# aptos-labs/keyless-zk-proofs

Measured on AMD Instinct MI355X. Metric: BN254 G1 MSM points/s @2^20 (Groth16 prover hot path), higher is better.
Workload: dtype u64 column accumulators over 9 x 29-bit limbs (256-bit Montgomery integers, v_mad_u64_u32); 1 GPU; BN254 G1 Pippenger MSM, 2^20 random scalars/points per GPU, result XYZZ on host; points_per_gpu=1048576, bases=reference format (Montgomery affine), converted inside every step

## Files before the change

include/k16.h:

```cpp
#ifndef K16_H
#define K16_H

#include <stddef.h>
#include <stdint.h>

#ifdef __cplusplus
extern "C" {
#endif

enum {
    K16_OK             = 0,
    K16_ERR_NO_DEVICE  = -1,
    K16_ERR_HIP        = -2,
    K16_ERR_ARG        = -3,
    K16_ERR_IO         = -4,
    K16_ERR_FORMAT     = -5,
    K16_ERR_CURVE      = -6,
    K16_ERR_BUFFER     = -7,
    K16_ERR_NOMEM      = -8
};

enum { K16_G1 = 0, K16_G2 = 1 };
enum { K16_FQ = 0, K16_FR = 1 };
enum { K16_FQ9 = 2, K16_FR9 = 3, K16_FQ2N = 4,
       K16_FQ2H = 5  };
enum { K16_G1_ENG9 = 2, K16_G2_ENG2N = 3, K16_G2_PAIR = 4  };
#define K16_OP_BOUND_A(k) ((k) << 8)
#define K16_OP_BOUND_B(k) ((k) << 12)
enum { K16_OP_ADD = 0, K16_OP_SUB, K16_OP_NEG, K16_OP_MUL, K16_OP_SQR, K16_OP_TOMONT, K16_OP_FROMMONT,
       K16_OP_LAZY_ADDMUL, K16_OP_LAZY_SUBMUL };
enum { K16_PT_ADD = 0, K16_PT_MADD, K16_PT_DBL,
       K16_PT_MADD_ACC };

typedef struct k16_ctx    k16_ctx;
typedef struct k16_prover k16_prover;

int         k16_runtime_hw_queues(int n);
int         k16_device_count(void);
int         k16_host_threads(void);

int         k16_ctx_create(int device, k16_ctx** out);
int         k16_ctx_create_ex(int device, int stream_offset, k16_ctx** out);
void        k16_ctx_destroy(k16_ctx* ctx);
const char* k16_last_error(const k16_ctx* ctx);
enum { K16_OPT_PIPELINED_MSM = 1, K16_OPT_GRAPHS = 2, K16_OPT_SHARED_GPU = 3, K16_OPT_YIELDING_WAITS = 4 };
int         k16_ctx_set_option(k16_ctx* ctx, int option, int value);
int         k16_sync(k16_ctx* ctx);
void*       k16_stream(k16_ctx* ctx);

int k16_dev_alloc(k16_ctx* ctx, size_t bytes, void** dptr);
int k16_dev_free(k16_ctx* ctx, void* dptr);
int k16_h2d(k16_ctx* ctx, void* dptr, const void* hptr, size_t bytes);
int k16_d2h(k16_ctx* ctx, void* hptr, const void* dptr, size_t bytes);
int k16_host_register(k16_ctx* ctx, void* hptr, size_t bytes);
int k16_host_unregister(k16_ctx* ctx, void* hptr);

int k16_timer_start(k16_ctx* ctx);
int k16_timer_stop(k16_ctx* ctx, float* elapsed_ms);
int k16_kernel_stats_enable(k16_ctx* ctx, int on);
int k16_kernel_stats_reset(k16_ctx* ctx);
int k16_kernel_stats_get(k16_ctx* ctx, const char* name, uint64_t* launches, double* total_ms);

int k16_msm(k16_ctx* ctx, int group, const void* d_bases, const void* d_scalars, uint64_t n, void* h_out_xyzz,
            void* h_out_affine);
int k16_msm_host(k16_ctx* ctx, int group, const void* h_bases, const void* h_scalars, uint64_t n, void* h_out_xyzz,
                 void* h_out_affine);
int k16_msm_enqueue(k16_ctx* ctx, int group, const void* d_bases, const void* d_scalars, uint64_t n);
int k16_msm_finish(k16_ctx* ctx, void* h_out_xyzz, void* h_out_affine);
int k16_msm_finish_group(k16_ctx* ctx, int group, void* h_out_xyzz, void* h_out_affine);
int k16_msm_pending(k16_ctx* ctx);
int k16_msm_abort_all(k16_ctx* ctx);
int k16_msm_bases_prepare(k16_ctx* ctx, int group, const void* d_bases, uint64_t n, void* d_out);
int k16_msm_enqueue_prepared(k16_ctx* ctx, int group, const void* d_prepared, const void* d_scalars, uint64_t n);
int k16_msm_fixed_base_info(uint64_t n, unsigned* c, uint64_t* table_rows);
int k16_msm_fixed_base_prepare(k16_ctx* ctx, int group, const void* d_bases, uint64_t n, void* d_table);
int k16_msm_enqueue_fixed_base(k16_ctx* ctx, int group, const void* d_table, const void* d_scalars, uint64_t n);
typedef struct k16_scalar_classes k16_scalar_classes;
int  k16_msm_zero_row_mask(k16_ctx* ctx, int group, const void* d_rows, uint64_t n, void* d_mask);
int  k16_scalar_classes_create(k16_ctx* ctx, uint64_t max_n, int max_sets, k16_scalar_classes** out);
void k16_scalar_classes_destroy(k16_scalar_classes* cls);
int  k16_scalar_classes_build(k16_ctx* ctx, k16_scalar_classes* cls, const void* d_scalars, uint64_t n,
                              const void* const* d_zero_masks, int n_sets, int64_t n_wide_bound);
int  k16_scalar_classes_counts(k16_ctx* ctx, const k16_scalar_classes* cls, uint32_t* out);
int  k16_msm_enqueue_classified(k16_ctx* ctx, int group, const void* d_prepared, const k16_scalar_classes* cls, int set);
int  k16_msm_set_zero_row_mask(k16_ctx* ctx, const void* d_mask);
int  k16_msm_sort_from_lane(k16_ctx* ctx, int lane, int derive);
#define K16_MSM_LANES 4
int k16_msm_set_lane(k16_ctx* ctx, int lane);
int k16_msm_set_window_bits(k16_ctx* ctx, unsigned c);

typedef struct k16_msm_shards k16_msm_shards;
int         k16_msm_sharded_create(const int* devices, int n_devices, int group, uint64_t n, k16_msm_shards** out);
void        k16_msm_sharded_destroy(k16_msm_shards* s);
int         k16_msm_sharded_count(const k16_msm_shards* s);
int         k16_msm_sharded_range(const k16_msm_shards* s, int shard, uint64_t* lo, uint64_t* hi);
k16_ctx*    k16_msm_sharded_ctx(k16_msm_shards* s, int shard);
const char* k16_msm_sharded_last_error(const k16_msm_shards* s);
int         k16_msm_sharded_set_bases(k16_msm_shards* s, const void* h_bases);
int         k16_msm_sharded_set_bases_device(k16_msm_shards* s, int shard, const void* d_slice);
int         k16_msm_sharded_run(k16_msm_shards* s, const void* h_scalars, void* h_out_xyzz, void* h_out_affine);
int         k16_msm_sharded_run_device(k16_msm_shards* s, const void* const* d_scalars, void* h_out_xyzz, void* h_out_affine);
int         k16_msm_sharded_set_piece_rows(k16_msm_shards* s, uint64_t host_rows, uint64_t device_rows);
int         k16_msm_sharded_last_ms(const k16_msm_shards* s, double* shards_ms, double* fold_ms, double* total_ms);
typedef struct k16_rank_comm k16_rank_comm;
int         k16_rank_comm_unique_id(void* out128);
const char* k16_rank_comm_load_error(void);
int         k16_rank_comm_create(k16_ctx* ctx, int rank, int world, const void* unique_id128, k16_rank_comm** out);
void        k16_rank_comm_destroy(k16_rank_comm* c);
int         k16_rank_comm_allgather_fold(k16_rank_comm* c, int group, const void* h_partial_xyzz, void* h_out_xyzz,
                                         void* h_out_affine);
int         k16_rank_comm_allgather_start(k16_rank_comm* c, int group, const void* h_partial_xyzz);
int         k16_rank_comm_allgather_finish(k16_rank_comm* c, void* h_out_xyzz, void* h_out_affine);

int k16_points_sum(int group, const void* h_parts_xyzz, uint64_t count, void* h_out_xyzz, void* h_out_affine);

int k16_ntt(k16_ctx* ctx, void* d_a, uint64_t n, uint64_t max_domain, int inverse);
int k16_ntt_host(k16_ctx* ctx, void* h_a, uint64_t n, uint64_t max_domain, int inverse);

int k16_synth_points(k16_ctx* ctx, int group, uint64_t start, uint64_t n, void* d_out_affine);
int k16_synth_points_scalars(k16_ctx* ctx, int group, const void* d_scalars, uint64_t n, void* d_out_affine);

int k16_field_op_vec(k16_ctx* ctx, int field, int op, const void* h_a, const void* h_b, void* h_r, uint64_t n);
int k16_point_op_vec(k16_ctx* ctx, int group, int op, const void* h_p1, const void* h_p2, void* h_r, uint64_t n);
int k16_coop_exec(k16_ctx* ctx, const uint8_t* step_class, uint64_t n_steps, const uint64_t* words ,
                  const uint32_t* terms, uint64_t n_terms, uint32_t n_const, uint32_t n_slots, const uint32_t* out_slot ,
                  const uint32_t* const9, const void* h_inputs, uint64_t n, void* h_out);

int  k16_prover_create(k16_ctx* ctx, const char* zkey_path, k16_prover** out);
int  k16_prover_create_mem(k16_ctx* ctx, const void* zkey_bytes, size_t zkey_size, k16_prover** out);
int  k16_prover_create_shared(k16_ctx* ctx, const k16_prover* other, k16_prover** out);
void k16_prover_destroy(k16_prover* p);
int  k16_prover_info(const k16_prover* p, uint32_t* n_vars, uint32_t* n_public, uint32_t* domain_size,
                     uint64_t* n_coefs);
int  k16_prover_prove_file(k16_prover* p, const char* wtns_path, const uint8_t* r_std, const uint8_t* s_std,
                           char* out_json, size_t cap, float* device_ms);
int  k16_prover_prove_file_timed(k16_prover* p, const char* wtns_path, const uint8_t* r_std, const uint8_t* s_std,
                                 char* out_json, size_t cap, float* device_ms, float* prove_wall_ms);
int  k16_prover_prove_mem(k16_prover* p, const void* h_wtns, uint64_t n_vars, const uint8_t* r_std,
                          const uint8_t* s_std, char* out_json, size_t cap, float* device_ms);
int  k16_prover_compact_buffers(k16_prover* p, uint8_t** narrow, uint32_t** wide_idx, uint8_t** wide_val, uint64_t* wide_cap);
int  k16_prover_prove_compact(k16_prover* p, uint64_t n_wide, const uint8_t* r_std, const uint8_t* s_std, char* out_json,
                              size_t cap, float* device_ms);
int  k16_fullprover_prove_mem(const void* fullprover, const void* wtns_values, uint64_t n_values, char* out_json, size_t cap,
                              int* prover_time_ms);
int  k16_fullprover_compact_lease(const void* fullprover, void** lease, uint8_t** narrow, uint32_t** wide_idx,
                                  uint8_t** wide_val, uint64_t* wide_cap, uint32_t* n_vars);
int  k16_fullprover_prove_compact(const void* fullprover, void* lease, uint64_t n_wide, char* out_json, size_t cap,
                                  int* prover_time_ms);
int  k16_fullprover_compact_cancel(const void* fullprover, void* lease);
int  k16_prover_last_h(k16_prover* p, void* h_out);
int  k16_prover_warmup_status(const k16_prover* p);

typedef struct k16_vk k16_vk;
int  k16_vk_create(k16_ctx* ctx, const void* alpha1_g1, const void* beta2_g2, const void* gamma2_g2, const void* delta2_g2,
                   const void* ic_g1, uint32_t n_ic, k16_vk** out);
void k16_vk_destroy(k16_vk* vk);
int  k16_verify_batch(k16_ctx* ctx, const k16_vk* vk, const void* h_proofs, const void* h_inputs, uint64_t n,
                      uint8_t* h_out_ok);
int  k16_verify_coop_gt(k16_ctx* ctx, const k16_vk* vk, const void* h_proofs, const void* h_inputs, uint64_t n, void* h_out_gt);
int  k16_pairing_vec(k16_ctx* ctx, const void* h_g1, const void* h_g2, uint64_t n, void* h_out_gt);

enum { K16_PT_OK = 0, K16_PT_NONCANONICAL = 1, K16_PT_OFF_CURVE = 2, K16_PT_NOT_IN_SUBGROUP = 3 };
enum { K16_VERIFY_PAIRING_MISMATCH = 4 };
int  k16_points_check(k16_ctx* ctx, int group, const void* h_points, uint64_t n, uint8_t* h_status);
int  k16_verify_batch_checked(k16_ctx* ctx, const k16_vk* vk, const void* h_proofs, const void* h_inputs, uint64_t n,
                              uint8_t* h_out_ok, uint8_t* h_out_reason);
#define K16_VERIFY_FOLD_MIN 2049
int  k16_verify_batch_folded(k16_ctx* ctx, const k16_vk* vk, const void* h_proofs, const void* h_inputs, uint64_t n,
                             uint8_t* h_out_ok, uint8_t* h_out_reason, uint8_t* out_folded);
int  k16_verify_fold_gt(k16_ctx* ctx, const k16_vk* vk, const void* h_proofs, const void* h_inputs, uint64_t n,
                        const void* h_weights, void* h_out_gt);
int  k16_vk_create_from_zkey(k16_ctx* ctx, const void* zkey, size_t size, k16_vk** out);
// ... 103 lines not shown
```

keyless-zk-proofs_amd/csrc/ctx.h:

```cpp
#pragma once
#include <hip/hip_runtime.h>
#include <map>
#include <mutex>
#include <new>
#include <exception>
#include <tuple>
#include <string>
#include <vector>
#include <stdint.h>
#include "../../include/k16.h"
#include "bn254_curve.h"
#include "bn254_fq9.h"

#include <atomic>
#include <condition_variable>
#include <functional>
#include <thread>

#include "host_pool.h"

#ifndef K16_CHAIN_PRIO
#define K16_CHAIN_PRIO 1
#endif

struct k16_devbuf {
    void*  p     = nullptr;
    size_t bytes = 0;
};

struct k16_kstat {
    uint64_t launches = 0;
    double   total_ms = 0;
};

struct k16_ntt_table {
    uint32_t  s      = 0;
    k16::Fr*  roots  = nullptr;
    uint32_t* roots9 = nullptr;
    uint32_t* stage9 = nullptr;
    k16::Fr   pow2inv[34];
    k16::Fq9  pow2inv9[34];
};

struct k16_tuning {
    bool     atomic_sort = false, b_sort = false, b_derive = false, classes = false, no_warmup = false, fused_hscalars = false;
    bool     b2_first = false;
    bool     trace = false, trace_enq = false, trace_host = false, verify_no_coop = false, verify_coop_trace = false;
    int      seg = 0;
    uint64_t verify_coop_max = 2048;
    static k16_tuning from_env();
};

struct k16_ctx {
    int         device = 0;
    k16_tuning  tune;
    hipStream_t stream = nullptr;
    hipEvent_t  ev_a = nullptr, ev_b = nullptr;
    std::vector<hipEvent_t> ks_pool;
    std::vector<std::pair<std::string, size_t>> ks_pending;
    size_t      ks_used = 0;
    int         stats_on = 0;
    std::map<std::string, k16_kstat> stats;
    std::string err;
    unsigned    forced_c = 0;

    static constexpr int N_LANES = 4;
    struct Lane {
        hipStream_t stream = nullptr;
        k16_devbuf  ws_counts, ws_offsets, ws_cursor, ws_sorted, ws_segoff, ws_segbucket, ws_partial, ws_big,
            ws_lvl_a, ws_lvl_b, ws_lvl_c, ws_lvl_d, ws_scan, ws_conv, ws_narrow;
        struct GraphEntry {
            int            state = 0;
            hipGraphExec_t exec  = nullptr;
        };
        typedef std::tuple<int, const void*, uint64_t, unsigned, unsigned, unsigned, int> GraphKey;
        std::map<GraphKey, GraphEntry> graphs;
        uint64_t                       graphs_gen = 0;
        hipEvent_t  sort_done = nullptr;
        hipEvent_t  acc_done  = nullptr;
        const void* sorted_scalars = nullptr;
        uint64_t    sorted_n = 0;
        unsigned    sorted_c = 0;
        const uint64_t* sorted_skip = nullptr;
        bool        sorted_plain_partition = false;
    };
    Lane lanes[N_LANES];
    int  cur_lane = 0;
    std::vector<hipStream_t> placeholder_streams;
    bool yielding_waits = false;
    void* pinned = nullptr;
    void* pinned_dev = nullptr;
    size_t pinned_bytes = 0;

    static constexpr int    PEND_SLOTS = 8;
    static constexpr size_t SLOT_BYTES = 128 * 1024;
    struct Pend {
        int      group = -1;
        unsigned c = 0, w = 0, nbits = 0, mlog = 0;
        bool     flat = false;
        uint64_t n = 0;
        int      slot = 0;
        unsigned narrow = 0;
        const struct k16_scalar_classes* cls = nullptr;
        bool     cls_overflow = false;
    };
    static constexpr size_t NARROW_OFF = SLOT_BYTES - 4096;
    std::mutex ring_mu;
    std::mutex verify_mu;
    Pend       pend[PEND_SLOTS];
    int        pend_head = 0, pend_count = 0;
    int        pend_reserved = 0;
    hipEvent_t pend_ev[PEND_SLOTS] = {};
    int        enq_slot = 0;
    unsigned   pend_mlog = 0;
    unsigned   pend_nbits = 0;
    unsigned   pend_wr = 0;

    bool        reuse_sort = false;
    unsigned    forced_seg = 0;
    bool        graphs_on = false;
    bool        capturing = false;
    uint64_t    ws_gen = 0;
    int         reuse_sort_lane = -1;
    const uint32_t* remap_next = nullptr;
    const uint64_t* skip_next = nullptr;
    const uint64_t* acc_skip_next = nullptr;
    int             derive_lane   = -1;
    unsigned        ntt_wg_per_cu = 4;
    const void*     hs_next[3]    = {nullptr, nullptr, nullptr};
    bool        serialize_acc = false;
    hipEvent_t  last_acc_done = nullptr;
    unsigned    wsum_mlog_cap = 3;

    std::map<uint32_t, k16_ntt_table> ntt_tables;
    bool                              parallel_combine = false;

    void*      gen_table[2] = {nullptr, nullptr};
    k16_devbuf gen_scratch;
};
struct k16_scalar_classes {
    static constexpr int MAX_SETS = 4, BITS = 8;
    k16_ctx*   ctx      = nullptr;
    uint64_t   cap_n    = 0;
    int        max_sets = 0, n_sets = 0;
    uint64_t   n        = 0;
    uint64_t   n_wide   = 0;
    uint32_t*  d_cnt    = nullptr;
    uint32_t*  d_lists  = nullptr;
    uint32_t*  d_wide_idx     = nullptr;
    uint8_t*   d_wide_scalars = nullptr;
    uint32_t*  h_flags  = nullptr;
    uint32_t*  h_flags_dev = nullptr;
    hipEvent_t built    = nullptr;
};

k16_host_pool* k16_ctx_pool(k16_ctx* ctx);

hipStream_t k16_lane_stream(k16_ctx* ctx, int lane);
hipError_t k16_event_wait(k16_ctx* ctx, hipEvent_t ev);

#define K16_HIP(ctx, call)                                                                         \
    do {                                                                                           \
        hipError_t e_ = (call);                                                                    \
        if (e_ != hipSuccess) {                                                                    \
            (ctx)->err = std::string(#call) + ": " + hipGetErrorString(e_);                        \
            return K16_ERR_HIP;                                                                    \
        }                                                                                          \
    } while (0)

int k16_ws_reserve(k16_ctx* ctx, k16_devbuf& b, size_t bytes);

template <class F>
inline int k16_guard(k16_ctx* ctx, F&& body) noexcept
{
    try {
        return body();
    } catch (const std::bad_alloc&) {
        try {
            if (ctx) ctx->err = "out of host memory";
        } catch (...) {
        }
        return K16_ERR_NOMEM;
    } catch (const std::exception& e) {
        try {
            if (ctx) ctx->err = std::string("internal error: ") + e.what();
        } catch (...) {
        }
        return K16_ERR_HIP;
    } catch (...) {
        return K16_ERR_HIP;
    }
}
template <class F>
inline void k16_guard_void(F&& body) noexcept
{
    try {
        body();
    } catch (...) {
    }
}

void k16_stats_begin(k16_ctx* ctx, const char* name, hipStream_t st);
void k16_stats_end(k16_ctx* ctx, hipStream_t st);
int  k16_stats_resolve(k16_ctx* ctx);

struct k16_stat_scope {
    k16_ctx*    ctx;
    bool        on;
    hipStream_t st;
    k16_stat_scope(k16_ctx* c, const char* n, hipStream_t s = nullptr)
// ... 29 lines not shown
```

keyless-zk-proofs_amd/csrc/ctx.hip:

```cpp
#include <stdio.h>
#include <stdlib.h>
#include <sched.h>
#include <string.h>
#include <algorithm>
#include <atomic>
#include <chrono>
#include <thread>
#include "ctx.h"
#include "bn254_fq2pair.h"
#include "bn254_fq9.h"

using namespace k16;

int k16_ws_reserve(k16_ctx* ctx, k16_devbuf& b, size_t bytes)
{
    if (b.bytes >= bytes) return K16_OK;
    if (b.p) {
        K16_HIP(ctx, hipDeviceSynchronize());
        K16_HIP(ctx, hipFree(b.p));
        b.p     = nullptr;
        b.bytes = 0;
    }
    size_t want = bytes + bytes / 8 + 4096;
    K16_HIP(ctx, hipMalloc(&b.p, want));
// ... 17 lines not shown
        (void)hipGetLastError();
        return 0;
    }
    return n < 0 ? 0 : n;
}

k16_tuning k16_tuning::from_env()
{
    k16_tuning t;
    auto on  = [](const char* n) { return getenv(n) != nullptr; };
    auto onv = [](const char* n) { const char* e = getenv(n); return e && atoi(e) != 0; };
    t.atomic_sort        = on("K16_ATOMIC_SORT");
    t.b_sort             = onv("K16_B_SORT");
    t.b_derive           = onv("K16_B_DERIVE");
    t.classes            = onv("K16_CLASSES");
    t.no_warmup          = on("K16_NO_WARMUP");
    t.fused_hscalars     = on("K16_FUSED_HSCALARS");
    t.b2_first           = on("K16_B2_FIRST");
    t.trace              = on("K16_TRACE");
    t.trace_enq          = on("K16_TRACE_ENQ");
    t.trace_host         = on("K16_TRACE_HOST");
    t.verify_no_coop     = on("K16_VERIFY_NO_COOP");
    t.verify_coop_trace  = on("K16_VERIFY_COOP_TRACE");
    if (const char* e = getenv("K16_SEG")) t.seg = atoi(e);
    if (const char* e = getenv("K16_VERIFY_COOP_MAX")) t.verify_coop_max = strtoull(e, nullptr, 10);
    return t;
}

extern "C" int k16_ctx_create(int device, k16_ctx** out) { return k16_ctx_create_ex(device, 0, out); }

extern "C" int k16_ctx_create_ex(int device, int stream_offset, k16_ctx** out)
{
    return k16_guard(nullptr, [&]() -> int {
    if (stream_offset < 0 || stream_offset > 7) return K16_ERR_ARG;
    if (!out) return K16_ERR_ARG;
    *out  = nullptr;
    int n = 0;
    if (hipGetDeviceCount(&n) != hipSuccess || n <= 0 || device < 0 || device >= n) return K16_ERR_NO_DEVICE;
    if (hipSetDevice(device) != hipSuccess) return K16_ERR_NO_DEVICE;
    k16_ctx* c = new k16_ctx();
    c->device  = device;
    c->tune    = k16_tuning::from_env();
    for (int k = 0; k < (stream_offset & 7); k++) {
        hipStream_t ph = nullptr;
        if (hipStreamCreateWithFlags(&ph, hipStreamNonBlocking) == hipSuccess) c->placeholder_streams.push_back(ph);
    }
    bool lanes_ok = true;
    for (int i = 0; i < k16_ctx::N_LANES; i++)
        lanes_ok = lanes_ok && (i > 0 || hipStreamCreateWithFlags(&c->lanes[i].stream, hipStreamNonBlocking) == hipSuccess) &&
                   hipEventCreateWithFlags(&c->lanes[i].sort_done, hipEventDisableTiming) == hipSuccess &&
                   hipEventCreateWithFlags(&c->lanes[i].acc_done, hipEventDisableTiming) == hipSuccess;
    c->stream = c->lanes[0].stream;
    if (!lanes_ok ||
        hipEventCreate(&c->ev_a) != hipSuccess || hipEventCreate(&c->ev_b) != hipSuccess) {
        delete c;
        return K16_ERR_NO_DEVICE;
    }
    c->pinned_bytes = k16_ctx::PEND_SLOTS * k16_ctx::SLOT_BYTES + 65536;
    if (hipHostMalloc(&c->pinned, c->pinned_bytes, hipHostMallocMapped | hipHostMallocCoherent) != hipSuccess ||
        hipHostGetDevicePointer(&c->pinned_dev, c->pinned, 0) != hipSuccess) {
        delete c;
        return K16_ERR_NO_DEVICE;
    }
    for (int i = 0; i < k16_ctx::PEND_SLOTS; i++)
        if (hipEventCreateWithFlags(&c->pend_ev[i], hipEventDisableTiming) != hipSuccess) {
            delete c;
            return K16_ERR_NO_DEVICE;
        }
    *out = c;
    return K16_OK;
    });
}

extern "C" void k16_ctx_destroy(k16_ctx* c)
{
    k16_guard_void([&]() {
    if (!c) return;
    (void)hipSetDevice(c->device);
    (void)hipStreamSynchronize(c->stream);
    (void)hipDeviceSynchronize();
    for (auto& L : c->lanes) {
        k16_devbuf* bufs[] = {&L.ws_counts, &L.ws_offsets, &L.ws_cursor, &L.ws_sorted, &L.ws_segoff, &L.ws_segbucket,
                              &L.ws_partial, &L.ws_big, &L.ws_lvl_a, &L.ws_lvl_b, &L.ws_lvl_c,
                              &L.ws_lvl_d, &L.ws_scan, &L.ws_conv, &L.ws_narrow};
        for (auto* b : bufs)
            if (b->p) (void)hipFree(b->p);
    }
    for (auto& kv : c->ntt_tables)
        if (kv.second.roots) (void)hipFree(kv.second.roots);
    for (auto& kv : c->ntt_tables)
        if (kv.second.roots9) (void)hipFree(kv.second.roots9);
    for (auto& kv : c->ntt_tables)
        if (kv.second.stage9) (void)hipFree(kv.second.stage9);
    for (void* t : c->gen_table)
        if (t) (void)hipFree(t);
    if (c->gen_scratch.p) (void)hipFree(c->gen_scratch.p);
    for (hipStream_t ph : c->placeholder_streams) (void)hipStreamDestroy(ph);
    if (c->pinned) (void)hipHostFree(c->pinned);
    for (int i = 0; i < k16_ctx::PEND_SLOTS; i++)
        if (c->pend_ev[i]) (void)hipEventDestroy(c->pend_ev[i]);
    (void)hipEventDestroy(c->ev_a);
    (void)hipEventDestroy(c->ev_b);
    for (hipEvent_t e : c->ks_pool) (void)hipEventDestroy(e);
    for (auto& L : c->lanes) {
        for (auto& kv : L.graphs)
            if (kv.second.exec) (void)hipGraphExecDestroy(kv.second.exec);
        if (L.sort_done) (void)hipEventDestroy(L.sort_done);
        if (L.acc_done) (void)hipEventDestroy(L.acc_done);
        if (L.stream && (&L == &c->lanes[0] || L.stream != c->lanes[0].stream)) (void)hipStreamDestroy(L.stream);
    }
    delete c;
    });
}

static k16_host_pool* g_host_pool       = nullptr;
static bool           g_host_pool_tried = false;
k16_host_pool* k16_ctx_pool(k16_ctx*)
{
    static std::mutex mu;
    std::lock_guard<std::mutex> lk(mu);
    if (g_host_pool || g_host_pool_tried) return g_host_pool;
    g_host_pool_tried = true;
    unsigned    want = 0;
    const char* e    = getenv("K16_HOST_THREADS");
    if (!e) e = getenv("K16_UPLOAD_THREADS");
    if (e) {
        want = (unsigned)std::max(0, std::min(32, atoi(e)));
    } else {
        cpu_set_t set;
        unsigned  n = 1;
        if (sched_getaffinity(0, sizeof set, &set) == 0) n = (unsigned)CPU_COUNT(&set);
        want = std::max(1u, std::min(12u, n * 3 / 4));
    }
    if (want < 2) return nullptr;
    try {
        g_host_pool = new k16_host_pool(want - 1);
    } catch (...) {
        g_host_pool = nullptr;
    }
    return g_host_pool;
}
extern "C" int k16_host_threads(void)
{
    return g_host_pool ? (int)g_host_pool->workers.size() : 0;
}

hipStream_t k16_lane_stream(k16_ctx* ctx, int lane)
{
    k16_ctx::Lane& L = ctx->lanes[lane];
    if (!L.stream) {
        (void)hipSetDevice(ctx->device);
        if (hipStreamCreateWithFlags(&L.stream, hipStreamNonBlocking) != hipSuccess) {
            ctx->err = "hipStreamCreate (MSM lane)";
            L.stream = ctx->stream;
        }
    }
    return L.stream;
}

hipError_t k16_event_wait(k16_ctx* ctx, hipEvent_t ev)
{
    if (!ctx->yielding_waits) return hipEventSynchronize(ev);
    for (unsigned spins = 0;; spins++) {
        const hipError_t q = hipEventQuery(ev);
        if (q != hipErrorNotReady) return q;
        if (spins < 8)
            std::this_thread::yield();
// ... 583 lines not shown
```

keyless-zk-proofs_amd/csrc/msm_api.hip:

```cpp
#include <string.h>
#include <algorithm>
#include <chrono>
#include <string>
#include <vector>
#include <functional>
#include "ctx.h"
#include "bn254_fq9.h"

using namespace k16;

int k16_msm_enqueue_g1(k16_ctx* ctx, const void* d_bases, const void* d_scalars, uint64_t n, unsigned c, int prepared);
int k16_msm_enqueue_g2(k16_ctx* ctx, const void* d_bases, const void* d_scalars, uint64_t n, unsigned c, int prepared);
int k16_msm_prepare_g1(k16_ctx* ctx, const void* d_bases, uint64_t n, void* d_out, hipStream_t st);
int k16_msm_prepare_g2(k16_ctx* ctx, const void* d_bases, uint64_t n, void* d_out, hipStream_t st);
int k16_msm_fixed_tables_g1(k16_ctx* ctx, const void* d_bases, uint64_t n, unsigned c, unsigned W, void* d_table);
int k16_msm_enqueue_fixed_g1(k16_ctx* ctx, const void* d_table, const void* d_scalars, uint64_t n, unsigned c);
int k16_msm_enqueue_classified_g1(k16_ctx* ctx, const void* d_rows, const k16_scalar_classes* cls, int set, unsigned c, bool* has_wide, int phase);
int k16_msm_enqueue_classified_g2(k16_ctx* ctx, const void* d_rows, const k16_scalar_classes* cls, int set, unsigned c, bool* has_wide, int phase);

namespace {
constexpr unsigned MAX_C = 16;
constexpr unsigned MIN_C = 4;
inline unsigned n_windows(unsigned c) { return (256 + c - 1) / c + 1; }

unsigned choose_c(const k16_ctx* ctx, uint64_t n)
{
    if (ctx->forced_c >= MIN_C && ctx->forced_c <= MAX_C) return ctx->forced_c;
    unsigned lg = 0;
    while ((n >> (lg + 1)) != 0) lg++;
    int c = (int)lg - (lg >= 18 ? 3 : 4);
    if (c < (int)MIN_C) c = MIN_C;
    if (c > (int)MAX_C) c = MAX_C;
    return (unsigned)c;
}

template <class F>
Xyzz<F> window_value_host(const Xyzz<F>* tw, unsigned nbits, unsigned mlog);
template <class F>
void window_values_host(k16_ctx* ctx, const Xyzz<F>* T, unsigned W, unsigned nbits, unsigned mlog, std::vector<Xyzz<F>>* out);
template <class F>
void horner_host(k16_ctx* ctx, const Xyzz<F>* T, unsigned W, unsigned c, unsigned nbits, unsigned mlog, Xyzz<F>* out)
{
    std::vector<Xyzz<F>> val;
    window_values_host<F>(ctx, T, W, nbits, mlog, &val);
    Xyzz<F> r = Xyzz<F>::zero();
    for (int w = (int)W - 1; w >= 0; w--) {
        for (unsigned k = 0; k < c; k++) r = pdbl(r);
        r = padd(r, val[w]);
    }
    *out = r;
}

template <class F>
Xyzz<F> window_value_host(const Xyzz<F>* tw, unsigned nbits, unsigned mlog)
{
    Xyzz<F> t = Xyzz<F>::zero();
    for (int b = (int)nbits - 1; b >= 0; b--) {
        t = pdbl(t);
        t = padd(t, tw[b]);
    }
    for (unsigned k = 0; k < mlog; k++) t = pdbl(t);
    t = padd(t, tw[nbits]);
    return padd(t, tw[nbits + 1]);
}
static thread_local const std::function<void(unsigned)>* g_window_prep = nullptr;
template <class F>
void window_values_host(k16_ctx* ctx, const Xyzz<F>* T, unsigned W, unsigned nbits, unsigned mlog, std::vector<Xyzz<F>>* out)
{
    out->resize(W);
    k16_host_pool* pool = (W >= 4 && ctx->parallel_combine) ? k16_ctx_pool(ctx) : nullptr;
    const std::function<void(unsigned)>* prep = g_window_prep;
    auto one = [&](unsigned w) {
        if (prep) (*prep)(w);
        (*out)[w] = window_value_host<F>(T + (size_t)w * (nbits + 2), nbits, mlog);
    };
    if (pool)
        pool->run(W, one);
    else
        for (unsigned w = 0; w < W; w++) one(w);
}

template <class F>
void flat_combine_host(k16_ctx* ctx, const Xyzz<F>* T, unsigned Wr, unsigned c, unsigned nbits, unsigned mlog, Xyzz<F>* out)
{
    std::vector<Xyzz<F>> val;
    window_values_host<F>(ctx, T, Wr, nbits, mlog, &val);
    Xyzz<F> total = Xyzz<F>::zero(), run = Xyzz<F>::zero(), wsum = Xyzz<F>::zero();
    for (int v = (int)Wr - 1; v >= 0; v--) {
        const Xyzz<F>* tw = T + (size_t)v * (nbits + 2);
        total = padd(total, val[v]);
        if (v > 0) {
            run  = padd(run, tw[nbits + 1]);
            wsum = padd(wsum, run);
        }
    }
    for (unsigned k = 0; k < nbits + mlog; k++) wsum = pdbl(wsum);
    (void)c;
    *out = padd(total, wsum);
}

unsigned fixed_base_c(uint64_t n)
// ... 104 lines not shown
    if (!ctx) return K16_ERR_ARG;
    ctx->skip_next = (const uint64_t*)d_mask;
    return K16_OK;
    });
}

extern "C" int k16_msm_sort_from_lane(k16_ctx* ctx, int lane, int derive)
{
    return k16_guard(ctx, [&]() -> int {
    if (!ctx || lane < 0 || lane >= k16_ctx::N_LANES) return K16_ERR_ARG;
    if (derive) {
        ctx->derive_lane = lane;
    } else {
        ctx->reuse_sort      = true;
        ctx->reuse_sort_lane = lane;
    }
    return K16_OK;
    });
}

extern "C" int k16_msm_set_window_bits(k16_ctx* ctx, unsigned c)
{
    return k16_guard(ctx, [&]() -> int {
    if (!ctx) return K16_ERR_ARG;
    if (c != 0 && (c < MIN_C || c > MAX_C)) return K16_ERR_ARG;
    ctx->forced_c = c;
    return K16_OK;
    });
}

namespace {
struct HostTimer {
    k16_ctx*                              c;
    const char*                           name;
    std::chrono::steady_clock::time_point t0;
    HostTimer(k16_ctx* cx, const char* nm) : c(cx), name(nm), t0(std::chrono::steady_clock::now()) {}
    ~HostTimer()
    {
        if (!c->stats_on) return;
        std::lock_guard<std::mutex> lk(c->ring_mu);
        auto&        st = c->stats[name];
        const double ms = std::chrono::duration<double, std::milli>(std::chrono::steady_clock::now() - t0).count();
        st.launches++;
        st.total_ms += ms;
        auto& mx = c->stats[std::string(name) + "_max"];
        mx.launches = 1;
        if (ms > mx.total_ms) mx.total_ms = ms;
    }
};
}

static int msm_enqueue_any(k16_ctx* ctx, int group, const void* d_bases, const void* d_scalars, uint64_t n, int prepared)
{
    OneShotGuard one_shot(ctx);
    if (!ctx || (group != K16_G1 && group != K16_G2)) return K16_ERR_ARG;
    HostTimer ht(ctx, "host_enqueue");
    K16_HIP(ctx, hipSetDevice(ctx->device));
    if (n >= (1ull << 32) / 80) {
        ctx->err = "k16_msm: n too large for one device call; shard it";
        return K16_ERR_ARG;
    }
    int idx;
    {
        std::lock_guard<std::mutex> lk(ctx->ring_mu);
        if (ctx->pend_count == k16_ctx::PEND_SLOTS) {
            ctx->err = "k16_msm_enqueue: too many MSMs in flight; call k16_msm_finish";
            return K16_ERR_ARG;
        }
        idx = (ctx->pend_head + ctx->pend_count) % k16_ctx::PEND_SLOTS;
    }
    k16_ctx::Pend pd;
    pd.group = group;
    pd.n     = n;
    pd.slot  = idx;
    int rc   = K16_OK;
    if (n != 0) {
        unsigned c    = choose_c(ctx, n);
        pd.c          = c;
        pd.w          = n_windows(c);
        ctx->enq_slot = idx;
        rc = group == K16_G1 ? k16_msm_enqueue_g1(ctx, d_bases, d_scalars, n, c, prepared)
                             : k16_msm_enqueue_g2(ctx, d_bases, d_scalars, n, c, prepared);
        if (rc) return rc;
        pd.nbits = ctx->pend_nbits;
        pd.mlog  = ctx->pend_mlog;
        K16_HIP(ctx, hipEventRecord(ctx->pend_ev[idx], k16_lane_stream(ctx, ctx->cur_lane)));
    }
    {
        std::lock_guard<std::mutex> lk(ctx->ring_mu);
        ctx->pend[idx] = pd;
        ctx->pend_count++;
    }
    return K16_OK;
}

extern "C" int k16_msm_enqueue(k16_ctx* ctx, int group, const void* d_bases, const void* d_scalars, uint64_t n)
{
    return k16_guard(ctx, [&]() -> int {
    return msm_enqueue_any(ctx, group, d_bases, d_scalars, n, 0);
    });
}
extern "C" int k16_msm_enqueue_prepared(k16_ctx* ctx, int group, const void* d_prepared, const void* d_scalars,
                                        uint64_t n)
{
    return k16_guard(ctx, [&]() -> int {
    return msm_enqueue_any(ctx, group, d_prepared, d_scalars, n, 1);
    });
}
int k16_msm_classified_phase(k16_ctx* ctx, int group, const void* d_prepared, const k16_scalar_classes* cls, int set, int phase)
{
    OneShotGuard one_shot(ctx);
    if (!ctx || !cls || cls->ctx != ctx || (group != K16_G1 && group != K16_G2) || set < 0 || set >= cls->n_sets ||
        (cls->n && !d_prepared))
        return K16_ERR_ARG;
    HostTimer ht(ctx, "host_enqueue");
    K16_HIP(ctx, hipSetDevice(ctx->device));
    int idx;
    {
        std::lock_guard<std::mutex> lk(ctx->ring_mu);
        const int ahead = phase == 1 ? ctx->pend_reserved : 0;
        if (ctx->pend_count + ahead >= k16_ctx::PEND_SLOTS || (phase == 2 && ctx->pend_reserved == 0)) {
            ctx->err = "k16_msm_enqueue: too many MSMs in flight; call k16_msm_finish";
            return K16_ERR_ARG;
        }
        idx = (ctx->pend_head + ctx->pend_count + ahead) % k16_ctx::PEND_SLOTS;
        if (phase == 1) ctx->pend_reserved++;
    }
    k16_ctx::Pend pd;
    pd.group = group;
    pd.n     = cls->n;
    pd.slot  = idx;
    if (cls->n != 0) {
        unsigned c = ctx->forced_c;
        if (c < MIN_C || c > MAX_C) {
            unsigned lg = 0;
            while ((std::max<uint64_t>(cls->n_wide, 1) >> (lg + 1)) != 0) lg++;
            c = (unsigned)std::min<int>(MAX_C, std::max<int>(MIN_C, (int)lg - 1));
        }
        ctx->enq_slot    = idx;
        bool has_wide    = false;
        int  rc = group == K16_G1 ? k16_msm_enqueue_classified_g1(ctx, d_prepared, cls, set, c, &has_wide, phase)
                                  : k16_msm_enqueue_classified_g2(ctx, d_prepared, cls, set, c, &has_wide, phase);
        if (rc) return rc;
        pd.cls    = cls;
        pd.narrow = k16_scalar_classes::BITS;
        if (has_wide) {
            pd.c     = c;
            pd.w     = n_windows(c);
            pd.nbits = ctx->pend_nbits;
            pd.mlog  = ctx->pend_mlog;
        }
        if (phase != 1) K16_HIP(ctx, hipEventRecord(ctx->pend_ev[idx], k16_lane_stream(ctx, ctx->cur_lane)));
    }
    if (phase != 1) {
        std::lock_guard<std::mutex> lk(ctx->ring_mu);
        ctx->pend[idx] = pd;
        ctx->pend_count++;
        if (phase == 2) ctx->pend_reserved--;
    }
    return K16_OK;
}
extern "C" int k16_msm_enqueue_classified(k16_ctx* ctx, int group, const void* d_prepared, const k16_scalar_classes* cls, int set)
{
    return k16_guard(ctx, [&]() -> int {
    if (ctx && ctx->pend_reserved) {
        ctx->err = "k16_msm_enqueue_classified: a split classified MSM is still open";
        return K16_ERR_ARG;
    }
    return k16_msm_classified_phase(ctx, group, d_prepared, cls, set, 0);
    });
}

extern "C" int k16_msm_bases_prepare(k16_ctx* ctx, int group, const void* d_bases, uint64_t n, void* d_out)
{
    return k16_guard(ctx, [&]() -> int {
    if (!ctx || (group != K16_G1 && group != K16_G2) || (n && (!d_bases || !d_out))) return K16_ERR_ARG;
// ... 117 lines not shown
            G2Aff a = to_affine(r);
            memcpy(h_out_affine, &a, sizeof a);
        }
    }
    return K16_OK;
}

extern "C" int k16_msm_finish(k16_ctx* ctx, void* h_out_xyzz, void* h_out_affine)
{
    return k16_guard(ctx, [&]() -> int {
    return msm_finish_any(ctx, -1, h_out_xyzz, h_out_affine);
    });
}
extern "C" int k16_msm_finish_group(k16_ctx* ctx, int group, void* h_out_xyzz, void* h_out_affine)
{
    return k16_guard(ctx, [&]() -> int {
    if (group != K16_G1 && group != K16_G2) return K16_ERR_ARG;
    return msm_finish_any(ctx, group, h_out_xyzz, h_out_affine);
    });
}
extern "C" int k16_msm_pending(k16_ctx* ctx)
{
    return k16_guard(ctx, [&]() -> int {
    if (!ctx) return K16_ERR_ARG;
    std::lock_guard<std::mutex> lk(ctx->ring_mu);
    return ctx->pend_count;
    });
}
extern "C" int k16_msm_abort_all(k16_ctx* ctx)
{
    return k16_guard(ctx, [&]() -> int {
    if (!ctx) return K16_ERR_ARG;
    int rc = K16_OK;
    while (k16_msm_pending(ctx) > 0) {
        int r = msm_finish_any(ctx, -1, nullptr, nullptr);
        if (r && !rc) rc = r;
    }
    ctx->reuse_sort      = false;
    ctx->reuse_sort_lane = -1;
    ctx->cur_lane        = 0;
    ctx->forced_seg      = 0;
    ctx->pend_reserved   = 0;
    ctx->remap_next      = nullptr;
    ctx->skip_next       = nullptr;
    ctx->acc_skip_next   = nullptr;
    ctx->derive_lane     = -1;
    ctx->hs_next[0] = ctx->hs_next[1] = ctx->hs_next[2] = nullptr;
    (void)hipSetDevice(ctx->device);
    for (auto& L : ctx->lanes)
        if (L.stream) (void)hipStreamSynchronize(L.stream);
    return rc;
    });
}

constexpr uint64_t MSM_CHUNK = 1ull << 24;

extern "C" int k16_msm(k16_ctx* ctx, int group, const void* d_bases, const void* d_scalars, uint64_t n,
                       void* h_out_xyzz, void* h_out_affine)
{
    return k16_guard(ctx, [&]() -> int {
    if (!ctx || (group != K16_G1 && group != K16_G2)) return K16_ERR_ARG;
    if (n <= MSM_CHUNK) {
        int rc = k16_msm_enqueue(ctx, group, d_bases, d_scalars, n);
        if (rc) return rc;
        return k16_msm_finish(ctx, h_out_xyzz, h_out_affine);
    }
    if (k16_msm_pending(ctx) != 0) {
        ctx->err = "k16_msm: a chunked (n > 2^24) call needs an empty MSM queue";
        return K16_ERR_ARG;
    }
    const size_t   pb       = group == K16_G1 ? sizeof(G1Aff) : sizeof(G2Aff);
    const size_t   xb       = group == K16_G1 ? sizeof(G1Xyzz) : sizeof(G2Xyzz);
    const uint64_t chunks   = (n + MSM_CHUNK - 1) / MSM_CHUNK;
    const int      saved    = ctx->cur_lane;
    std::vector<unsigned char> parts((size_t)chunks * xb);
    int      rc = K16_OK;
    uint64_t enq = 0, fin = 0;
    auto enqueue_next = [&]() -> int {
        const uint64_t lo = enq * MSM_CHUNK, cnt = std::min<uint64_t>(MSM_CHUNK, n - lo);
        ctx->cur_lane = (int)(enq % 2);
        enq++;
        return k16_msm_enqueue(ctx, group, (const char*)d_bases + lo * pb, (const char*)d_scalars + lo * 32, cnt);
    };
    rc = enqueue_next();
    while (!rc && fin < chunks) {
        if (enq < chunks) rc = enqueue_next();
        if (!rc) rc = k16_msm_finish(ctx, parts.data() + (size_t)fin * xb, nullptr);
        fin++;
    }
    ctx->cur_lane = saved;
    if (rc) {
        (void)k16_msm_abort_all(ctx);
        return rc;
    }
    return k16_points_sum(group, parts.data(), chunks, h_out_xyzz, h_out_affine);
    });
}

extern "C" int k16_msm_host(k16_ctx* ctx, int group, const void* h_bases, const void* h_scalars, uint64_t n,
                            void* h_out_xyzz, void* h_out_affine)
{
    return k16_guard(ctx, [&]() -> int {
    if (!ctx || (group != K16_G1 && group != K16_G2)) return K16_ERR_ARG;
    if (n == 0) return k16_msm(ctx, group, nullptr, nullptr, 0, h_out_xyzz, h_out_affine);
    size_t pb = (size_t)n * (group == K16_G1 ? sizeof(G1Aff) : sizeof(G2Aff));
    void * db = nullptr, *ds = nullptr;
    K16_HIP(ctx, hipMalloc(&db, pb));
    hipError_t e = hipMalloc(&ds, (size_t)n * 32);
    if (e != hipSuccess) {
        (void)hipFree(db);
        ctx->err = "hipMalloc scalars";
        return K16_ERR_HIP;
    }
    int rc = K16_OK;
    if (hipMemcpyAsync(db, h_bases, pb, hipMemcpyHostToDevice, ctx->stream) != hipSuccess ||
        hipMemcpyAsync(ds, h_scalars, (size_t)n * 32, hipMemcpyHostToDevice, ctx->stream) != hipSuccess) {
        ctx->err = "hipMemcpyAsync h2d";
        rc       = K16_ERR_HIP;
    }
    if (!rc && hipStreamSynchronize(ctx->stream) != hipSuccess) rc = K16_ERR_HIP;
    if (!rc) rc = k16_msm(ctx, group, db, ds, n, h_out_xyzz, h_out_affine);
    (void)hipDeviceSynchronize();
    (void)hipFree(db);
    (void)hipFree(ds);
    return rc;
    });
}

extern "C" int k16_points_sum(int group, const void* h_parts, uint64_t count, void* h_out_xyzz, void* h_out_affine)
{
    return k16_guard(nullptr, [&]() -> int {
    if (group == K16_G1) {
        G1Xyzz acc = G1Xyzz::zero();
        for (uint64_t i = 0; i < count; i++) {
            G1Xyzz p;
            memcpy(&p, (const char*)h_parts + i * sizeof p, sizeof p);
            acc = padd(acc, p);
        }
        if (h_out_xyzz) memcpy(h_out_xyzz, &acc, sizeof acc);
        if (h_out_affine) {
            G1Aff a = to_affine(acc);
            memcpy(h_out_affine, &a, sizeof a);
        }
        return K16_OK;
    }
    if (group == K16_G2) {
        G2Xyzz acc = G2Xyzz::zero();
        for (uint64_t i = 0; i < count; i++) {
            G2Xyzz p;
            memcpy(&p, (const char*)h_parts + i * sizeof p, sizeof p);
            acc = padd(acc, p);
        }
        if (h_out_xyzz) memcpy(h_out_xyzz, &acc, sizeof acc);
        if (h_out_affine) {
            G2Aff a = to_affine(acc);
            memcpy(h_out_affine, &a, sizeof a);
        }
        return K16_OK;
    }
    return K16_ERR_ARG;
    });
}
```

keyless-zk-proofs_amd/csrc/msm_g1.hip:

```cpp
#define K16_FMUL_CHAINS 1
#include <algorithm>
#include "msm_kernels.inc"

int k16_msm_prepare_g1(k16_ctx* ctx, const void* d_bases, uint64_t n, void* d_out, hipStream_t st)
{
    if (!st) st = ctx->stream;
    if (n == 0) return K16_OK;
    hipLaunchKernelGGL(k_convert_bases, dim3((unsigned)((n + 255) / 256)), dim3(256), 0, st,
                       (const k16::G1Aff*)d_bases, (k16::G1Aff*)d_out, n);
    K16_HIP(ctx, hipGetLastError());
    return K16_OK;
}
int k16_msm_enqueue_g1(k16_ctx* ctx, const void* d_bases, const void* d_scalars, uint64_t n, unsigned c, int prepared)
{
    const k16::G1Aff* rows = (const k16::G1Aff*)d_bases;
    const void*       conv_in = nullptr;
    if (!prepared) {
        k16_ctx::Lane& L = ctx->lanes[ctx->cur_lane];
        int rc = k16_ws_reserve(ctx, L.ws_conv, (size_t)n * sizeof(k16::G1Aff));
        if (rc) return rc;
        rows = (const k16::G1Aff*)L.ws_conv.p;
        const bool fuse = n <= (1u << 24) && !ctx->reuse_sort && ctx->derive_lane < 0 && !ctx->graphs_on && !ctx->tune.atomic_sort;
        if (fuse)
            conv_in = d_bases;
        else if ((rc = k16_msm_prepare_g1(ctx, d_bases, n, L.ws_conv.p, k16_lane_stream(ctx, ctx->cur_lane))))
            return rc;
    }
    return msm_enqueue_t<Eng9>(ctx, rows, d_scalars, n, c, false, conv_in);
}

namespace {
__global__ void __launch_bounds__(128) k_window_table_next(const k16::G1Aff* __restrict__ prev, k16::G1Aff* __restrict__ next,
                                                           uint64_t n, unsigned c)
{
    using namespace k16;
    const uint64_t i = (uint64_t)blockIdx.x * blockDim.x + threadIdx.x;
    if (i >= n) return;
    Aff<Fq> w = load_vec(&prev[i]);
    Aff9    a{fq9_unpack(w.x.v), fq9_unpack(w.y.v)};
    Aff<Fq> o;
    for (int k = 0; k < 8; k++) o.x.v[k] = o.y.v[k] = 0;
    if (!a.is_zero()) {
        Xyzz9 p = pdbl_aff9(a);
#pragma clang loop unroll(disable)
        for (unsigned k = 1; k < c; k++) p = pdbl9(p);
        if (!p.is_zero()) {
            Fq9 t = finv9(fmul9(p.zz, p.zzz));
            Fq9 x = fmul9(p.x, fmul9(t, p.zzz));
            Fq9 y = fmul9(p.y, fmul9(t, p.zz));
            fq9_pack(o.x.v, x);
            fq9_pack(o.y.v, y);
        }
    }
    store_vec(&next[i], o);
}
}

int k16_msm_fixed_tables_g1(k16_ctx* ctx, const void* d_bases, uint64_t n, unsigned c, unsigned W, void* d_table)
{
    hipStream_t st = ctx->stream;
    int         rc = k16_msm_prepare_g1(ctx, d_bases, n, d_table, st);
    if (rc || n == 0) return rc;
    k16::G1Aff* t = (k16::G1Aff*)d_table;
    for (unsigned w = 1; w < W; w++)
        hipLaunchKernelGGL(k_window_table_next, dim3((unsigned)((n + 127) / 128)), dim3(128), 0, st, t + (size_t)(w - 1) * n,
                           t + (size_t)w * n, n, c);
    K16_HIP(ctx, hipGetLastError());
    return K16_OK;
}
int k16_msm_enqueue_fixed_g1(k16_ctx* ctx, const void* d_table, const void* d_scalars, uint64_t n, unsigned c)
{
    return msm_enqueue_t<Eng9>(ctx, (const k16::G1Aff*)d_table, d_scalars, n, c, true);
}
int k16_msm_enqueue_classified_g1(k16_ctx* ctx, const void* d_rows, const k16_scalar_classes* cls, int set, unsigned c,
                                  bool* has_wide, int phase)
{
    return msm_enqueue_classified_t<Eng9>(ctx, (const k16::G1Aff*)d_rows, cls, set, c, has_wide, phase);
}
```

keyless-zk-proofs_amd/csrc/msm_kernels.inc:

```
#include <stdio.h>
#include <chrono>
#include <stdlib.h>
#include <string.h>
#include "ctx.h"
#include "bn254_fq2pair.h"
#include "bn254_fq9.h"

using namespace k16;

namespace {

constexpr unsigned MIN_SEG   = 32;
constexpr unsigned MAX_SEG   = 1024;
constexpr unsigned FOLD_SMALL = 16;
constexpr unsigned WSUM_MLOG_MAX = 5;
constexpr unsigned MAX_C     = 16;
constexpr unsigned MIN_C     = 4;

__host__ __device__ inline unsigned n_windows(unsigned c) { return (256 + c - 1) / c + 1; }

__device__ __forceinline__ void k16_lds_sync()
{
    asm volatile("s_waitcnt lgkmcnt(0)" ::: "memory");
    __syncthreads();
}

__device__ __forceinline__ void k16_short_kernel_prio()
{
#ifndef K16_NO_SETPRIO
#ifndef K16_SHORT_PRIO
#define K16_SHORT_PRIO 3
#endif
    __builtin_amdgcn_s_setprio(K16_SHORT_PRIO);
#endif
}

#ifndef K16_G2_ACC_PRIO
#define K16_G2_ACC_PRIO 0
#endif
#ifndef K16_G1_ACC_PRIO
#define K16_G1_ACC_PRIO 0
#endif
template <class E>
__device__ __forceinline__ void k16_acc_prio()
{
    if constexpr (E::ALPP == 2) {
        if (K16_G2_ACC_PRIO) __builtin_amdgcn_s_setprio(K16_G2_ACC_PRIO);
    } else {
        if (K16_G1_ACC_PRIO) __builtin_amdgcn_s_setprio(K16_G1_ACC_PRIO);
    }
}

template <unsigned C>
__device__ __forceinline__ uint32_t digit_of(const uint32_t (&k)[8], unsigned w)
{
    const unsigned bit = w * C;
    const unsigned wd  = bit >> 5;
    const unsigned sh  = bit & 31;
    uint64_t       v   = k[wd];
    if (wd + 1 < 8) v |= (uint64_t)k[wd + 1] << 32;
    return (uint32_t)(v >> sh) & ((1u << C) - 1u);
}

template <unsigned C, class Fn>
__device__ __forceinline__ void for_signed_digits(const uint32_t (&k)[8], Fn f)
{
    constexpr unsigned W    = (256 + C - 1) / C;
    constexpr uint32_t HALF = 1u << (C - 1), FULL = 1u << C;
    uint32_t           carry = 0;
#pragma unroll
    for (unsigned w = 0; w < W; w++) {
        const uint32_t v   = digit_of<C>(k, w) + carry;
        const uint32_t neg = v > HALF ? 1u : 0u;
        carry              = neg;
        const uint32_t m   = neg ? FULL - v : v;
        if (m) f(w, m - 1u, neg);
    }
    if (carry) f(W, 0u, 0u);
}

template <unsigned C, class Fn>
__device__ __forceinline__ void for_signed_digits_flat(const uint32_t (&k)[8], Fn f)
{
    constexpr unsigned W    = (257 + C - 1) / C;
    constexpr uint32_t HALF = 1u << (C - 1), FULL = 1u << C;
    uint32_t           carry = 0;
#pragma unroll
    for (unsigned w = 0; w < W; w++) {
        const uint32_t raw = w * C < 256 ? digit_of<C>(k, w) : 0u;
        const uint32_t v   = raw + carry;
        const uint32_t neg = v > HALF ? 1u : 0u;
        carry              = neg;
        const uint32_t m   = neg ? FULL - v : v;
        if (m) f(w, m - 1u, neg);
    }
}

template <unsigned C, bool SCATTER>
__global__ void __launch_bounds__(256) k_digits(const uint4* __restrict__ scalars, uint64_t n,
                                                uint32_t* __restrict__ counts_or_cursor,
                                                uint32_t* __restrict__ sorted, const uint32_t* __restrict__ remap)
{
    k16_short_kernel_prio();
    for (uint64_t i = (uint64_t)blockIdx.x * blockDim.x + threadIdx.x; i < n; i += (uint64_t)gridDim.x * blockDim.x) {
        uint4    lo = scalars[2 * i], hi = scalars[2 * i + 1];
        uint32_t k[8] = {lo.x, lo.y, lo.z, lo.w, hi.x, hi.y, hi.z, hi.w};
        for_signed_digits<C>(k, [&](unsigned w, uint32_t m1, uint32_t neg) {
            uint32_t key = (w << (C - 1)) + m1;
            if (SCATTER) {
                uint32_t pos = atomicAdd(&counts_or_cursor[key], 1u);
                sorted[pos]  = (neg << 31) | (remap ? remap[i] : (uint32_t)i);
            } else {
                atomicAdd(&counts_or_cursor[key], 1u);
            }
        });
    }
}

template <class T>
__device__ __forceinline__ T load_vec(const T* __restrict__ p)
{
    static_assert(sizeof(T) % 16 == 0, "16-byte granularity");
    T            r;
    const uint4* s = reinterpret_cast<const uint4*>(p);
    uint4*       d = reinterpret_cast<uint4*>(&r);
#pragma unroll
    for (unsigned i = 0; i < sizeof(T) / 16; i++) d[i] = s[i];
    return r;
}
template <class T>
__device__ __forceinline__ void store_vec(T* __restrict__ p, const T& v)
{
    static_assert(sizeof(T) % 16 == 0, "16-byte granularity");
    uint4*       d = reinterpret_cast<uint4*>(p);
    const uint4* s = reinterpret_cast<const uint4*>(&v);
#pragma unroll
    for (unsigned i = 0; i < sizeof(T) / 16; i++) d[i] = s[i];
}

#ifndef K16_PART_TILE
#define K16_PART_TILE 2048
#endif
constexpr unsigned PART_TILE = K16_PART_TILE;

template <unsigned CC>
struct PartCfg {
    static constexpr unsigned C   = CC;
    static constexpr unsigned W   = (256 + C - 1) / C + 1;
    static constexpr unsigned BB  = C - 1;
    static constexpr unsigned LO  = BB > 7 ? 7 : BB;
    static constexpr unsigned LO4 = LO;
    static constexpr unsigned HI  = BB - LO;
    static constexpr unsigned NB1 = W << HI;
    static constexpr unsigned SHIFT = 24;
    static constexpr bool     FLAT  = false;
    static constexpr unsigned TILE  = PART_TILE;
};
template <unsigned CC>
struct PartCfgFlat {
    static constexpr unsigned C   = CC;
    static constexpr unsigned W   = (257 + C - 1) / C;
    static constexpr unsigned BB  = C - 1;
    static constexpr unsigned LO  = 6;
    static constexpr unsigned LO4 = LO;
    static constexpr unsigned HI  = BB - LO;
    static constexpr unsigned NB1 = 1u << HI;
    static constexpr unsigned SHIFT = 25;
    static constexpr bool     FLAT  = true;
    static constexpr unsigned TILE  = PART_TILE;
};

constexpr unsigned PART_SLICE = 8192;
template <bool SLICES>
__device__ __forceinline__ void part_scan_lds(const uint32_t* __restrict__ gcount, uint32_t nb1, uint32_t* __restrict__ out,
                                              uint32_t* __restrict__ sh , uint32_t* __restrict__ total)
{
    const unsigned per = (nb1 + 255) / 256;
    uint32_t       sum = 0;
    for (unsigned j = 0; j < per; j++) {
        unsigned b = threadIdx.x * per + j;
        uint32_t v = b < nb1 ? gcount[b] : 0u;
        sum += SLICES ? (v + PART_SLICE - 1) / PART_SLICE : v;
    }
    sh[threadIdx.x] = sum;
    k16_lds_sync();
    for (unsigned o = 1; o < 256; o <<= 1) {
        uint32_t t = threadIdx.x >= o ? sh[threadIdx.x - o] : 0u;
        k16_lds_sync();
        sh[threadIdx.x] += t;
        k16_lds_sync();
    }
    uint32_t run = sh[threadIdx.x] - sum;
    if (threadIdx.x == 255) *total = sh[255];
    for (unsigned j = 0; j < per; j++) {
        unsigned b = threadIdx.x * per + j;
        if (b < nb1) {
            out[b]     = run;
            uint32_t v = gcount[b];
            run += SLICES ? (v + PART_SLICE - 1) / PART_SLICE : v;
        }
    }
    k16_lds_sync();
}

__device__ __forceinline__ k16::Fr hs_scalar(const k16::Fr* __restrict__ a, const k16::Fr* __restrict__ b,
                                             const k16::Fr* __restrict__ c, uint64_t i)
{
    auto ld9 = [](const k16::Fr* p) -> k16::Fr9 {
        const uint4* s4 = reinterpret_cast<const uint4*>(p);
        const uint4  x = s4[0], y = s4[1];
        const uint32_t w[8] = {x.x, x.y, x.z, x.w, y.x, y.y, y.z, y.w};
        return k16::fr9_load(w);
    };
    return k16::fr9_to_standard(k16::frsub9(k16::frmul9(ld9(&a[i]), ld9(&b[i])), ld9(&c[i])));
}
__global__ void __launch_bounds__(256) k_hs_fill(uint4* __restrict__ scalars, uint64_t n, const k16::Fr* __restrict__ a,
                                                 const k16::Fr* __restrict__ b, const k16::Fr* __restrict__ c)
{
    const uint64_t i = (uint64_t)blockIdx.x * blockDim.x + threadIdx.x;
    if (i >= n) return;
    const k16::Fr v = hs_scalar(a, b, c, i);
    scalars[2 * i]     = make_uint4(v.v[0], v.v[1], v.v[2], v.v[3]);
    scalars[2 * i + 1] = make_uint4(v.v[4], v.v[5], v.v[6], v.v[7]);
}

template <class P, bool SCATTER, bool CONV = false, bool HS = false>
__global__ void __launch_bounds__(256) k_part(const uint4* __restrict__ scalars, uint64_t n, uint32_t* __restrict__ g,
                                              uint32_t* __restrict__ part, const k16::Aff<k16::Fq>* __restrict__ conv_in,
                                              k16::Aff<k16::Fq>* __restrict__ conv_out, const uint32_t* __restrict__ gcount,
                                              uint32_t* __restrict__ gstart, uint32_t* __restrict__ gslice,
                                              const uint64_t* __restrict__ skip = nullptr,
                                              const k16::Fr* __restrict__ hs_a = nullptr, const k16::Fr* __restrict__ hs_b = nullptr,
                                              const k16::Fr* __restrict__ hs_c = nullptr)
{
    static_assert(!HS || (!SCATTER && !CONV), "the H scalars are formed by the plain counting pass");
    k16_short_kernel_prio();
    extern __shared__ uint32_t  part_lds[];
    __shared__ uint32_t         sh[256];
    __shared__ uint32_t         s_total;
    constexpr unsigned          HW = (P::NB1 + 1) / 2;
    uint32_t*                   hist = part_lds;
    uint32_t*                   base = part_lds + HW;
    auto hadd = [&](uint32_t b) -> uint32_t {
        const unsigned sh16 = (b & 1u) << 4;
        return (atomicAdd(&hist[b >> 1], 1u << sh16) >> sh16) & 0xffffu;
    };
    auto hget = [&](uint32_t b) -> uint32_t { return (hist[b >> 1] >> ((b & 1u) << 4)) & 0xffffu; };
    const uint32_t              ntiles = (uint32_t)((n + P::TILE - 1) / P::TILE);
    auto bin_of = [](unsigned w, uint32_t m1) -> uint32_t { return P::FLAT ? (m1 >> P::LO) : ((w << P::HI) + (m1 >> P::LO)); };
    auto digits = [](const uint32_t (&k)[8], auto f) {
        if constexpr (P::FLAT)
            for_signed_digits_flat<P::C>(k, f);
        else
            for_signed_digits<P::C>(k, f);
    };
    if (SCATTER) {
        if (blockIdx.x == 0) {
            part_scan_lds<true>(gcount, P::NB1, base, sh, &s_total);
            for (unsigned b = threadIdx.x; b < P::NB1; b += blockDim.x) gslice[b] = base[b];
            if (threadIdx.x == 0) gslice[P::NB1] = s_total;
            k16_lds_sync();
        }
        part_scan_lds<false>(gcount, P::NB1, base, sh, &s_total);
        if (blockIdx.x == 0) {
            for (unsigned b = threadIdx.x; b < P::NB1; b += blockDim.x) gstart[b] = base[b];
            if (threadIdx.x == 0) gstart[P::NB1] = s_total;
        }
    }
    if constexpr (SCATTER) {
        constexpr unsigned PPT = P::TILE / 256;
        constexpr unsigned BPT = (P::NB1 + 255) / 256;
        const uint32_t     tile = blockIdx.x;
        uint4              sc[PPT][2];
#pragma unroll
        for (unsigned p = 0; p < PPT; p++) {
            const uint64_t i = (uint64_t)tile * P::TILE + p * 256 + threadIdx.x;
            if (i < n && !(skip && ((skip[i >> 6] >> (i & 63u)) & 1ull))) {
                sc[p][0] = scalars[2 * i];
                sc[p][1] = scalars[2 * i + 1];
            } else {
                sc[p][0] = sc[p][1] = make_uint4(0u, 0u, 0u, 0u);
            }
        }
        for (unsigned b = threadIdx.x; b < HW; b += blockDim.x) hist[b] = 0;
        k16_lds_sync();
#pragma unroll
        for (unsigned p = 0; p < PPT; p++) {
            uint32_t k[8] = {sc[p][0].x, sc[p][0].y, sc[p][0].z, sc[p][0].w, sc[p][1].x, sc[p][1].y, sc[p][1].z, sc[p][1].w};
            digits(k, [&](unsigned w, uint32_t m1, uint32_t) { (void)hadd(bin_of(w, m1)); });
        }
        k16_lds_sync();
        uint32_t got[BPT];
#pragma unroll
        for (unsigned j = 0; j < BPT; j++) {
            const unsigned b = threadIdx.x + j * 256;
            uint32_t       h = b < P::NB1 ? hget(b) : 0u;
            got[j]           = h ? atomicAdd(&g[b], h) : 0u;
        }
#pragma unroll
        for (unsigned j = 0; j < BPT; j++) {
            const unsigned b = threadIdx.x + j * 256;
            if (b < P::NB1) base[b] += got[j];
        }
        k16_lds_sync();
        for (unsigned b = threadIdx.x; b < HW; b += blockDim.x) hist[b] = 0;
        k16_lds_sync();
#pragma unroll
        for (unsigned p = 0; p < PPT; p++) {
            const uint64_t i = (uint64_t)tile * P::TILE + p * 256 + threadIdx.x;
            uint32_t k[8] = {sc[p][0].x, sc[p][0].y, sc[p][0].z, sc[p][0].w, sc[p][1].x, sc[p][1].y, sc[p][1].z, sc[p][1].w};
            digits(k, [&](unsigned w, uint32_t m1, uint32_t neg) {
                uint32_t b   = bin_of(w, m1);
                uint32_t r   = hadd(b);
                uint32_t row = P::FLAT ? (uint32_t)(w * n + i) : (uint32_t)i;
                part[base[b] + r] = (neg << 31) | ((m1 & ((1u << P::LO) - 1u)) << P::SHIFT) | row;
            });
        }
        return;
    }
    for (uint32_t tile = blockIdx.x; tile < ntiles; tile += gridDim.x) {
        for (unsigned b = threadIdx.x; b < HW; b += blockDim.x) hist[b] = 0;
        k16_lds_sync();
        for (unsigned p = 0; p < P::TILE / 256; p++) {
            const uint64_t i = (uint64_t)tile * P::TILE + p * 256 + threadIdx.x;
            if (i >= n) break;
            uint4 lo, hi;
            if constexpr (HS) {
                const k16::Fr v = hs_scalar(hs_a, hs_b, hs_c, i);
                lo = make_uint4(v.v[0], v.v[1], v.v[2], v.v[3]);
                hi = make_uint4(v.v[4], v.v[5], v.v[6], v.v[7]);
                uint4* out = const_cast<uint4*>(scalars);
                out[2 * i]     = lo;
                out[2 * i + 1] = hi;
            } else {
                lo = scalars[2 * i];
                hi = scalars[2 * i + 1];
            }
            uint32_t k[8] = {lo.x, lo.y, lo.z, lo.w, hi.x, hi.y, hi.z, hi.w};
            if (!(skip && ((skip[i >> 6] >> (i & 63u)) & 1ull)))
                digits(k, [&](unsigned w, uint32_t m1, uint32_t) { (void)hadd(bin_of(w, m1)); });
            if constexpr (CONV) {
                k16::Aff<k16::Fq> a = load_vec(&conv_in[i]);
                k16::Aff9         c9 = k16::aff9_from_canonical(a);
                k16::Aff<k16::Fq> o;
                k16::fq9_pack(o.x.v, c9.x);
                k16::fq9_pack(o.y.v, c9.y);
                store_vec(&conv_out[i], o);
            }
        }
        k16_lds_sync();
        for (unsigned b = threadIdx.x; b < P::NB1; b += blockDim.x) {
            uint32_t h = hget(b);
            if (h) atomicAdd(&g[b], h);
        }
        k16_lds_sync();
    }
}

constexpr unsigned WC_THREADS = 1024;
__global__ void __launch_bounds__(WC_THREADS) k_bin_starts(const uint32_t* __restrict__ gcount, uint32_t nb1,
                                                          uint32_t* __restrict__ gstart, uint32_t* __restrict__ gslice)
{
    k16_short_kernel_prio();
    __shared__ uint32_t sa[WC_THREADS], sb[WC_THREADS];
    const unsigned per = (nb1 + WC_THREADS - 1) / WC_THREADS;
    uint32_t       a = 0, b = 0;
    for (unsigned j = 0; j < per; j++) {
        const unsigned i = threadIdx.x * per + j;
        const uint32_t v = i < nb1 ? gcount[i] : 0u;
        a += v;
        b += (v + PART_SLICE - 1) / PART_SLICE;
    }
    sa[threadIdx.x] = a;
    sb[threadIdx.x] = b;
    k16_lds_sync();
    for (unsigned o = 1; o < WC_THREADS; o <<= 1) {
        const uint32_t ta = threadIdx.x >= o ? sa[threadIdx.x - o] : 0u, tb = threadIdx.x >= o ? sb[threadIdx.x - o] : 0u;
        k16_lds_sync();
        sa[threadIdx.x] += ta;
        sb[threadIdx.x] += tb;
        k16_lds_sync();
    }
    uint32_t ra = sa[threadIdx.x] - a, rb = sb[threadIdx.x] - b;
    for (unsigned j = 0; j < per; j++) {
        const unsigned i = threadIdx.x * per + j;
        if (i < nb1) {
            gstart[i]        = ra;
            gslice[i]        = rb;
            const uint32_t v = gcount[i];
            ra += v;
            rb += (v + PART_SLICE - 1) / PART_SLICE;
        }
    }
    if (threadIdx.x == WC_THREADS - 1) {
        gstart[nb1] = sa[WC_THREADS - 1];
        gslice[nb1] = sb[WC_THREADS - 1];
    }
}

template <unsigned CC>
struct PartCfgFlat5 {
    static constexpr unsigned C   = CC;
    static constexpr unsigned W   = (257 + C - 1) / C;
    static constexpr unsigned BB  = C - 1;
    static constexpr unsigned LO  = 9;
    static constexpr unsigned LO4 = 6;
    static constexpr unsigned HI  = BB - LO;
    static constexpr unsigned NB1 = 1u << HI;
    static constexpr unsigned SHIFT = 25;
    static constexpr bool     FLAT  = true;
    static constexpr unsigned TILE  = PART_TILE;
#ifndef K16_ST_TILE_FLAT
#define K16_ST_TILE_FLAT 2048
#endif
    static constexpr unsigned ST_TILE = K16_ST_TILE_FLAT;
};
template <unsigned CC>
struct PartCfg5 {
    static constexpr unsigned C   = CC;
    static constexpr unsigned W   = (256 + C - 1) / C + 1;
    static constexpr unsigned BB  = C - 1;
    static constexpr unsigned LO  = BB > 9 ? 9 : BB;
    static constexpr unsigned LO4 = 7;
    static constexpr unsigned HI  = BB - LO;
    static constexpr unsigned NB1 = W << HI;
    static constexpr unsigned SHIFT = 24;
    static constexpr bool     FLAT  = false;
    static constexpr unsigned TILE  = PART_TILE;
    static constexpr unsigned ST_TILE = 1024;
};
constexpr unsigned ST_THREADS = 1024;
template <class P>
struct StageGeom {
    static constexpr unsigned CAP       = P::ST_TILE * P::W;
    static constexpr unsigned NBP       = (P::NB1 + ST_THREADS - 1) / ST_THREADS;
    static constexpr unsigned LDS_BYTES = (3 * P::NB1 + 1 + ST_THREADS + CAP) * 4 + ((CAP + 3) & ~3u);
};
template <class P>
__global__ void __launch_bounds__(ST_THREADS) k_part_stage(const uint4* __restrict__ scalars, uint64_t n, uint32_t* __restrict__ g,
                                                           uint32_t* __restrict__ part4, uint8_t* __restrict__ part1,
                                                           const uint32_t* __restrict__ gstart)
{
    k16_short_kernel_prio();
    typedef StageGeom<P>       G;
    extern __shared__ uint32_t st_lds[];
    uint32_t* cur  = st_lds;
    uint32_t* toff = cur + P::NB1;
    uint32_t* gdl  = toff + P::NB1 + 1;
    uint32_t* sh   = gdl + P::NB1;
    uint32_t* st4  = sh + ST_THREADS;
    uint8_t*  st1  = reinterpret_cast<uint8_t*>(st4 + G::CAP);
    constexpr unsigned PPT = P::ST_TILE / ST_THREADS;
    auto bin_of = [](unsigned w, uint32_t m1) -> uint32_t { return P::FLAT ? (m1 >> P::LO) : ((w << P::HI) + (m1 >> P::LO)); };
    auto digits = [](const uint32_t (&k)[8], auto f) {
        if constexpr (P::FLAT)
            for_signed_digits_flat<P::C>(k, f);
        else
            for_signed_digits<P::C>(k, f);
    };
    const uint32_t tile = blockIdx.x;
    uint4          sc[PPT][2];
#pragma unroll
    for (unsigned p = 0; p < PPT; p++) {
        const uint64_t i = (uint64_t)tile * P::ST_TILE + p * ST_THREADS + threadIdx.x;
        if (i < n) {
            sc[p][0] = scalars[2 * i];
            sc[p][1] = scalars[2 * i + 1];
        } else {
            sc[p][0] = sc[p][1] = make_uint4(0u, 0u, 0u, 0u);
        }
    }
    for (unsigned b = threadIdx.x; b < P::NB1; b += ST_THREADS) cur[b] = 0;
    k16_lds_sync();
#pragma unroll
    for (unsigned p = 0; p < PPT; p++) {
        uint32_t k[8] = {sc[p][0].x, sc[p][0].y, sc[p][0].z, sc[p][0].w, sc[p][1].x, sc[p][1].y, sc[p][1].z, sc[p][1].w};
        digits(k, [&](unsigned w, uint32_t m1, uint32_t) { atomicAdd(&cur[bin_of(w, m1)], 1u); });
    }
    k16_lds_sync();
    {
        uint32_t h[G::NBP], sum = 0;
#pragma unroll
        for (unsigned j = 0; j < G::NBP; j++) {
            const unsigned b = threadIdx.x * G::NBP + j;
            h[j]             = b < P::NB1 ? cur[b] : 0u;
            sum += h[j];
        }
        sh[threadIdx.x] = sum;
        k16_lds_sync();
        for (unsigned o = 1; o < ST_THREADS; o <<= 1) {
            const uint32_t t = threadIdx.x >= o ? sh[threadIdx.x - o] : 0u;
            k16_lds_sync();
            sh[threadIdx.x] += t;
            k16_lds_sync();
        }
        uint32_t run = sh[threadIdx.x] - sum;
        uint32_t got[G::NBP];
#pragma unroll
        for (unsigned j = 0; j < G::NBP; j++) {
            const unsigned b = threadIdx.x * G::NBP + j;
            got[j]           = (b < P::NB1 && h[j]) ? atomicAdd(&g[b], h[j]) : 0u;
        }
#pragma unroll
        for (unsigned j = 0; j < G::NBP; j++) {
            const unsigned b = threadIdx.x * G::NBP + j;
            if (b < P::NB1) {
                cur[b]  = run;
                toff[b] = run;
                gdl[b]  = gstart[b] + got[j];
                run += h[j];
            }
        }
        if (threadIdx.x == ST_THREADS - 1) toff[P::NB1] = sh[ST_THREADS - 1];
    }
    k16_lds_sync();
#pragma unroll
    for (unsigned p = 0; p < PPT; p++) {
        const uint64_t i = (uint64_t)tile * P::ST_TILE + p * ST_THREADS + threadIdx.x;
        uint32_t k[8] = {sc[p][0].x, sc[p][0].y, sc[p][0].z, sc[p][0].w, sc[p][1].x, sc[p][1].y, sc[p][1].z, sc[p][1].w};
        digits(k, [&](unsigned w, uint32_t m1, uint32_t neg) {
            const uint32_t pos = atomicAdd(&cur[bin_of(w, m1)], 1u);
            const uint32_t row = P::FLAT ? (uint32_t)(w * n + i) : (uint32_t)i;
            const uint32_t lo  = m1 & ((1u << P::LO) - 1u);
            st4[pos] = (neg << 31) | ((lo & ((1u << P::LO4) - 1u)) << P::SHIFT) | row;
            st1[pos] = (uint8_t)(lo >> P::LO4);
        });
    }
    k16_lds_sync();
    const unsigned hw = threadIdx.x >> 5, l32 = threadIdx.x & 31u;
    for (unsigned b = hw; b < P::NB1; b += ST_THREADS / 32) {
        const uint32_t lo = toff[b], len = toff[b + 1] - lo, dst = gdl[b];
        for (uint32_t k = l32; k < len; k += 32) {
            part4[dst + k] = st4[lo + k];
            part1[dst + k] = st1[lo + k];
        }
    }
}

template <class P, int MODE>
__global__ void __launch_bounds__(256) k_part_bins(const uint32_t* __restrict__ gstart, const uint32_t* __restrict__ gslice,
                                                   uint32_t nb1, const uint32_t* __restrict__ part,
                                                   uint32_t* __restrict__ counts_or_cursor, uint32_t* __restrict__ sorted,
                                                   const uint32_t* __restrict__ remap,
                                                   const uint8_t* __restrict__ side = nullptr, uint32_t small_cap = 0,
                                                   const uint64_t* __restrict__ drop = nullptr)
{
    k16_short_kernel_prio();
    constexpr unsigned  LON = 1u << P::LO;
    constexpr unsigned  HN  = LON > 256 ? LON : 256;
    constexpr bool      SIDE = LON > 128;
    constexpr unsigned  LO4  = P::LO4;
    __shared__ uint32_t h[HN], base[HN];
    __shared__ uint32_t s_bin;
    const uint32_t      g = blockIdx.x;
    if (g >= gslice[nb1]) return;
    if (threadIdx.x == 0) {
        uint32_t lo = 0, hi = nb1;
        if (g < nb1 && gslice[g] == g && gslice[g + 1] > g) {
            lo = g;
        } else {
            while (hi - lo > 1) {
                uint32_t mid = (lo + hi) >> 1;
                if (gslice[mid] <= g) lo = mid; else hi = mid;
            }
        }
        s_bin = lo;
    }
    for (unsigned t = threadIdx.x; t < HN; t += 256) h[t] = 0;
    k16_lds_sync();
    const uint32_t bin    = s_bin;
    if (small_cap && gstart[bin + 1] - gstart[bin] <= small_cap) return;
    const uint32_t s0  = gstart[bin] + (g - gslice[bin]) * PART_SLICE;
    const uint32_t s1  = min(s0 + PART_SLICE, gstart[bin + 1]);
    constexpr unsigned EPT = PART_SLICE / 256;
    uint32_t           ent[EPT];
    uint32_t           sdp[SIDE ? EPT / 4 : 1];
    uint32_t           dropped = 0;
    static_assert(EPT <= 32, "one bit per entry of a lane");
#pragma unroll
    for (unsigned k = 0; k < EPT; k++) {
        const uint32_t j = s0 + k * 256 + threadIdx.x;
        ent[k]           = j < s1 ? part[j] : 0xffffffffu;
    }
    if (drop) {
#pragma unroll
        for (unsigned k = 0; k < EPT; k++) {
            const uint32_t j  = s0 + k * 256 + threadIdx.x;
            const uint32_t pt = ent[k] & ((1u << P::SHIFT) - 1u);
            if (j < s1 && ((drop[pt >> 6] >> (pt & 63u)) & 1ull)) dropped |= 1u << k;
        }
    }
    if constexpr (SIDE) {
#pragma unroll
        for (unsigned k = 0; k < EPT / 4; k++) sdp[k] = 0;
#pragma unroll
        for (unsigned k = 0; k < EPT; k++) {
            const uint32_t j = s0 + k * 256 + threadIdx.x;
            if (j < s1) sdp[k >> 2] |= (uint32_t)side[j] << ((k & 3u) * 8);
        }
    }
    auto low_key = [&](unsigned k, uint32_t e) -> uint32_t {
        if constexpr (SIDE)
            return ((e >> P::SHIFT) & ((1u << LO4) - 1u)) | (((sdp[k >> 2] >> ((k & 3u) * 8)) & 0xffu) << LO4);
        else
            return (e >> P::SHIFT) & (LON - 1u);
// ... 872 lines not shown
            uint32_t        k2  = k + 1;
            while (k2 < R && !sel(k2)) k2++;
            if (k2 < R) nxt = E::tload(&src[lo | (k2 << p) | (hi << (p + rb))]);
            acc = E::tadd(acc, cur);
            k   = k2;
        }
    } else {
        for (uint32_t u = t; u < U; u += 256) {
            if (j < nbits && !((u >> j) & 1)) continue;
            acc = E::tadd(acc, E::tload(&src[u]));
        }
    }
    lds[threadIdx.x] = acc;
    k16_lds_sync();
    for (unsigned o = 128; o > 0; o >>= 1) {
        if (t < o) {
            typename E::TPt a = lds[threadIdx.x], b = lds[threadIdx.x + o * LPP];
            lds[threadIdx.x] = E::tadd(a, b);
        }
        k16_lds_sync();
    }
    if (t == 0) E::tstore(&T[blockIdx.x], lds[threadIdx.x]);
}

template <class Body>
int run_graph_section(k16_ctx* ctx, k16_ctx::Lane& L, hipStream_t st, const k16_ctx::Lane::GraphKey& key, Body body)
{
    if (!ctx->graphs_on) return body();
    if (L.graphs_gen != ctx->ws_gen) {
        for (auto& kv : L.graphs)
            if (kv.second.exec) (void)hipGraphExecDestroy(kv.second.exec);
        L.graphs.clear();
        L.graphs_gen = ctx->ws_gen;
    }
    k16_ctx::Lane::GraphEntry& ge = L.graphs[key];
    if (ge.state == 2) {
        K16_HIP(ctx, hipGraphLaunch(ge.exec, st));
        return K16_OK;
    }
    if (ge.state == 0) {
        const uint64_t gen = ctx->ws_gen;
        int            rc  = body();
        if (!rc && gen == ctx->ws_gen) ge.state = 1;
        return rc;
    }
    if (ge.state < 0) return body();
    if (hipStreamBeginCapture(st, hipStreamCaptureModeThreadLocal) != hipSuccess) {
        (void)hipGetLastError();
        ge.state = -1;
        return body();
    }
    ctx->capturing = true;
    int        rc  = body();
    hipGraph_t g   = nullptr;
    hipError_t e   = hipStreamEndCapture(st, &g);
    ctx->capturing = false;
    if (rc || e != hipSuccess || !g || hipGraphInstantiate(&ge.exec, g, nullptr, nullptr, 0) != hipSuccess) {
        (void)hipGetLastError();
        if (g) (void)hipGraphDestroy(g);
        ge.exec  = nullptr;
        ge.state = -1;
        return rc ? rc : body();
    }
    (void)hipGraphDestroy(g);
    ge.state = 2;
    K16_HIP(ctx, hipGraphLaunch(ge.exec, st));
    return K16_OK;
}

struct SortArgs {
    const void* d_scalars;
    uint64_t    n;
    unsigned    c, W;
    bool        flat;
    uint32_t    nb, seg, big_cap;
    size_t      max_segs, zr_words;
    uint32_t *  zr, *misc, *gcount, *gcursor, *seg_hist, *counts, *offsets, *cursor, *seg_off, *sorted, *scan_tmp, *big_list,
        *seg_bucket, *seg_order;
    const void* conv_in;
    void*       conv_out;
    const uint32_t* remap;
    const uint64_t* skip;
    const void*     hs[3];
};
constexpr size_t SORT_GS = 8208;

template <class Tick>
int msm_sort_launch(k16_ctx* ctx, k16_ctx::Lane& L, hipStream_t st, const SortArgs& a, Tick&& tick)
{
    int            rc;
    const void*    d_scalars = a.d_scalars;
    const uint64_t n = a.n;
    const unsigned c = a.c, W = a.W;
    const bool     flat = a.flat;
    const uint32_t nb = a.nb, seg = a.seg, big_cap = a.big_cap;
    const size_t   max_segs = a.max_segs, zr_words = a.zr_words;
    uint32_t *zr = a.zr, *misc = a.misc, *gcount = a.gcount, *gcursor = a.gcursor, *seg_hist = a.seg_hist, *counts = a.counts,
             *offsets = a.offsets, *cursor = a.cursor, *seg_off = a.seg_off, *sorted = a.sorted, *scan_tmp = a.scan_tmp,
             *big_list = a.big_list, *seg_bucket = a.seg_bucket, *seg_order = a.seg_order;
    const void* conv_in  = a.conv_in;
    void*       conv_out = a.conv_out;
    const uint32_t* remap = a.remap;
    const bool      use_part = flat || (n <= (1u << 24) && !ctx->tune.atomic_sort);
    const uint64_t* skip     = use_part ? a.skip : nullptr;
    constexpr size_t GS  = SORT_GS;
    {
        k16_stat_scope ss(ctx, "msm_sort", st);
        tick("pre");
        K16_HIP(ctx, hipMemsetAsync(zr, 0, zr_words * 4, st));
        tick("memset");
        const bool staged = use_part && !skip && n >= (1u << 16) && ((flat && c == 20) || (!flat && c == 16 && n < (1u << 24)));
        const bool hs_fused = a.hs[0] && staged && flat && !a.conv_in;
        if (a.hs[0] && !hs_fused)
            hipLaunchKernelGGL(k_hs_fill, dim3((unsigned)((n + 255) / 256)), dim3(256), 0, st, (uint4*)const_cast<void*>(d_scalars), n,
                               (const k16::Fr*)a.hs[0], (const k16::Fr*)a.hs[1], (const k16::Fr*)a.hs[2]);
        constexpr unsigned SCAN_BLK = SCAN_T * SCAN_PER_DEFAULT;
        const unsigned nblk = (nb + SCAN_BLK - 1) / SCAN_BLK;
        if (nblk > 4096) {
            ctx->err = "msm: too many buckets for the scan workspace";
            return K16_ERR_ARG;
        }
        const unsigned grid = (unsigned)std::min<uint64_t>((n + 255) / 256, 256 * 8);
        auto scans = [&]() {
            hipLaunchKernelGGL(k_scan2_totals<SCAN_PER_DEFAULT>, dim3(nblk), dim3(SCAN_T), 0, st, counts, nb, seg, scan_tmp);
            hipLaunchKernelGGL(k_scan2_apply<SCAN_PER_DEFAULT>, dim3(nblk), dim3(SCAN_T), 0, st, counts, nb, seg, scan_tmp, offsets, cursor,
                               seg_off, misc, big_list, big_cap, big_list + big_cap, big_list + big_cap + GIANT_CAP, seg_bucket,
                               seg_hist);
        };
        if (use_part) {
            if ((rc = k16_ws_reserve(ctx, L.ws_lvl_d, 2 * GS * 4 + (size_t)n * W * 5 + 64))) return rc;
            uint32_t* gstart = (uint32_t*)L.ws_lvl_d.p;
            uint32_t* gslice = gstart + GS;
            uint32_t* part   = gstart + 2 * GS;
#define K16_PART(CC) K16_PART_CFG(CC, PartCfg<CC>)
#define K16_PART_CFG(CC, CFG)                                                                                     \
    case CC: {                                                                                                   \
        const unsigned nb1   = CFG::NB1;                                                                         \
        const unsigned ntiles = (unsigned)((n + CFG::TILE - 1) / CFG::TILE);                                     \
        const unsigned pgrid  = std::min<unsigned>(ntiles, 256 * 4);                                             \
        const unsigned sgrid = nb1 + (unsigned)(((uint64_t)n * W) / PART_SLICE) + 1;                              \
        static_assert(CFG::NB1 + 1 <= GS, "partition tables too small");                                         \
        if (conv_in)                                                                                             \
            hipLaunchKernelGGL((k_part<CFG, false, true>), dim3(pgrid), dim3(256), ((nb1 + 1) / 2 + nb1) * 4, st,     \
                               (const uint4*)d_scalars, n, gcount, part, (const k16::Aff<k16::Fq>*)conv_in,            \
                               (k16::Aff<k16::Fq>*)conv_out, (const uint32_t*)nullptr, (uint32_t*)nullptr,             \
                               (uint32_t*)nullptr, skip);                                                                  \
        else                                                                                                     \
            hipLaunchKernelGGL((k_part<CFG, false, false>), dim3(pgrid), dim3(256), ((nb1 + 1) / 2 + nb1) * 4, st,    \
                               (const uint4*)d_scalars, n, gcount, part, (const k16::Aff<k16::Fq>*)nullptr,            \
                               (k16::Aff<k16::Fq>*)nullptr, (const uint32_t*)nullptr, (uint32_t*)nullptr,              \
                               (uint32_t*)nullptr, skip);                                                                  \
        hipLaunchKernelGGL((k_part<CFG, true>), dim3(ntiles), dim3(256), ((nb1 + 1) / 2 + nb1) * 4, st, (const uint4*)d_scalars, n, \
                           gcursor, part, (const k16::Aff<k16::Fq>*)nullptr, (k16::Aff<k16::Fq>*)nullptr,         \
                           (const uint32_t*)gcount, gstart, gslice, skip);                                              \
        hipLaunchKernelGGL((k_part_bins<CFG, 0>), dim3(sgrid), dim3(256), 0, st, gstart, gslice, nb1, part, counts, sorted, remap); \
        scans();                                                                                                 \
        hipLaunchKernelGGL((k_part_bins<CFG, 1>), dim3(sgrid), dim3(256), 0, st, gstart, gslice, nb1, part, cursor, sorted, remap); \
    } break;
#define K16_PART_STAGED(CFG)                                                                                      \
    {                                                                                                            \
        const unsigned nb1    = CFG::NB1;                                                                        \
        const unsigned ntiles = (unsigned)((n + CFG::TILE - 1) / CFG::TILE);                                     \
        const unsigned pgrid  = std::min<unsigned>(ntiles, 256 * 4);                                             \
        const unsigned sgrid  = nb1 + (unsigned)(((uint64_t)n * W) / PART_SLICE) + 1;                            \
        const unsigned stiles = (unsigned)((n + CFG::ST_TILE - 1) / CFG::ST_TILE);                               \
        const unsigned slds   = StageGeom<CFG>::LDS_BYTES;                                                       \
        static_assert(CFG::NB1 + 1 <= GS, "partition tables too small");                                         \
        static_assert(StageGeom<CFG>::LDS_BYTES <= 160 * 1024, "stage does not fit the LDS");                    \
        static bool st_attr = false;                                                                             \
        if (!st_attr) {                                                                                          \
            K16_HIP(ctx, hipFuncSetAttribute((const void*)k_part_stage<CFG>, hipFuncAttributeMaxDynamicSharedMemorySize, (int)slds)); \
            st_attr = true;                                                                                      \
        }                                                                                                        \
        uint8_t* part1 = (uint8_t*)(part + (size_t)n * W);                                                       \
        if (hs_fused)                                                                                            \
            hipLaunchKernelGGL((k_part<CFG, false, false, true>), dim3(pgrid), dim3(256), ((nb1 + 1) / 2 + nb1) * 4, st, \
                               (const uint4*)d_scalars, n, gcount, part, (const k16::Aff<k16::Fq>*)nullptr,       \
                               (k16::Aff<k16::Fq>*)nullptr, (const uint32_t*)nullptr, (uint32_t*)nullptr, (uint32_t*)nullptr, \
                               (const uint64_t*)nullptr, (const k16::Fr*)a.hs[0], (const k16::Fr*)a.hs[1],       \
                               (const k16::Fr*)a.hs[2]);                                                         \
        else if (conv_in)                                                                                        \
            hipLaunchKernelGGL((k_part<CFG, false, true>), dim3(pgrid), dim3(256), ((nb1 + 1) / 2 + nb1) * 4, st, \
                               (const uint4*)d_scalars, n, gcount, part, (const k16::Aff<k16::Fq>*)conv_in,       \
                               (k16::Aff<k16::Fq>*)conv_out, (const uint32_t*)nullptr, (uint32_t*)nullptr, (uint32_t*)nullptr); \
        else                                                                                                     \
        hipLaunchKernelGGL((k_part<CFG, false, false>), dim3(pgrid), dim3(256), ((nb1 + 1) / 2 + nb1) * 4, st,   \
                           (const uint4*)d_scalars, n, gcount, part, (const k16::Aff<k16::Fq>*)nullptr,           \
                           (k16::Aff<k16::Fq>*)nullptr, (const uint32_t*)nullptr, (uint32_t*)nullptr, (uint32_t*)nullptr); \
        hipLaunchKernelGGL(k_bin_starts, dim3(1), dim3(WC_THREADS), 0, st, (const uint32_t*)gcount, nb1, gstart, gslice); \
        hipLaunchKernelGGL((k_part_stage<CFG>), dim3(stiles), dim3(ST_THREADS), slds, st, (const uint4*)d_scalars, n, gcursor, \
                           part, part1, (const uint32_t*)gstart);                                                \
        static bool bs_attr = false;                                                                             \
        const unsigned blds = ((1u << CFG::LO) + BS_THREADS + BS_CAP) * 4;                                       \
        if (!bs_attr) {                                                                                          \
            K16_HIP(ctx, hipFuncSetAttribute((const void*)k_bins_stage<CFG>, hipFuncAttributeMaxDynamicSharedMemorySize, (int)blds)); \
            bs_attr = true;                                                                                      \
        }                                                                                                        \
        hipLaunchKernelGGL((k_bins_stage<CFG>), dim3(nb1), dim3(BS_THREADS), blds, st, (const uint32_t*)gstart, nb1,         \
                           (const uint32_t*)part, (const uint8_t*)part1, counts, sorted, remap);                 \
        hipLaunchKernelGGL((k_part_bins<CFG, 0>), dim3(sgrid), dim3(256), 0, st, gstart, gslice, nb1, part, counts, sorted,     \
                           remap, (const uint8_t*)part1, BS_CAP);                                                \
        scans();                                                                                                 \
        hipLaunchKernelGGL((k_part_bins<CFG, 1>), dim3(sgrid), dim3(256), 0, st, gstart, gslice, nb1, part, cursor, sorted,     \
                           remap, (const uint8_t*)part1, BS_CAP);                                                \
    }
            if (staged && flat) {
                K16_PART_STAGED(PartCfgFlat5<20>)
            } else if (staged) {
                K16_PART_STAGED(PartCfg5<16>)
            } else if (flat) {
                switch (c) {
                    K16_PART_CFG(12, PartCfgFlat<12>) K16_PART_CFG(14, PartCfgFlat<14>) K16_PART_CFG(16, PartCfgFlat<16>)
                    K16_PART_CFG(18, PartCfgFlat<18>) K16_PART_CFG(20, PartCfgFlat<20>)
                default: ctx->err = "unsupported fixed-base window size"; return K16_ERR_ARG;
                }
            } else {
                switch (c) {
                    K16_PART(4) K16_PART(5) K16_PART(6) K16_PART(7) K16_PART(8) K16_PART(9) K16_PART(10) K16_PART(11)
                    K16_PART(12) K16_PART(13) K16_PART(14) K16_PART(15) K16_PART(16)
                default: ctx->err = "unsupported window size"; return K16_ERR_ARG;
                }
            }
        } else {
#define K16_DIGITS(CC, SC, ARG0, ARG1)                                                                    \
    case CC: hipLaunchKernelGGL((k_digits<CC, SC>), dim3(grid), dim3(256), 0, st, (const uint4*)d_scalars, n, ARG0, ARG1, remap); break;
#define K16_DIGITS_ALL(SC, ARG0, ARG1)                                                                     \
    switch (c) {                                                                                           \
        K16_DIGITS(4, SC, ARG0, ARG1) K16_DIGITS(5, SC, ARG0, ARG1) K16_DIGITS(6, SC, ARG0, ARG1)          \
        K16_DIGITS(7, SC, ARG0, ARG1) K16_DIGITS(8, SC, ARG0, ARG1) K16_DIGITS(9, SC, ARG0, ARG1)          \
        K16_DIGITS(10, SC, ARG0, ARG1) K16_DIGITS(11, SC, ARG0, ARG1) K16_DIGITS(12, SC, ARG0, ARG1)       \
        K16_DIGITS(13, SC, ARG0, ARG1) K16_DIGITS(14, SC, ARG0, ARG1) K16_DIGITS(15, SC, ARG0, ARG1)       \
        K16_DIGITS(16, SC, ARG0, ARG1)                                                                     \
    default: ctx->err = "unsupported window size"; return K16_ERR_ARG;                                     \
    }
        K16_DIGITS_ALL(false, counts, (uint32_t*)nullptr)
        scans();
        K16_DIGITS_ALL(true, cursor, sorted)
        }
        tick("part+scan");
        const unsigned sgrid = (unsigned)std::min<size_t>((max_segs + 256 * SEG_PER_THREAD - 1) / (256 * SEG_PER_THREAD), 1024);
        hipLaunchKernelGGL(k_seg_scatter, dim3(sgrid), dim3(256), 0, st, offsets, seg_off, misc + 1, seg_bucket, seg_hist,
                           seg_hist + (MAX_SEG + 1), seg_order, seg);
        K16_HIP(ctx, hipGetLastError());
        return K16_OK;
    }
}

int msm_sort_plan(k16_ctx* ctx, k16_ctx::Lane& SL, const void* d_scalars, uint64_t n, unsigned c, bool flat, bool reuse,
                  const void* conv_in, void* conv_out, SortArgs* out)
{
    int            rc;
    const unsigned W  = flat ? (257 + c - 1) / c : n_windows(c);
    const uint32_t nb = flat ? (1u << (c - 1)) : (W << (c - 1));
    constexpr size_t GS     = SORT_GS;
    constexpr size_t ZR_HDR = (16 + 2 * GS + 2 * (MAX_SEG + 1) + 3) & ~(size_t)3;
    const size_t     zr_words = ZR_HDR + nb + 1;
    if (!reuse) {
        if ((rc = k16_ws_reserve(ctx, SL.ws_counts, zr_words * 4))) return rc;
        if ((rc = k16_ws_reserve(ctx, SL.ws_offsets, (size_t)(nb + 1) * 4))) return rc;
        if ((rc = k16_ws_reserve(ctx, SL.ws_cursor, (size_t)(nb + 1) * 4))) return rc;
        if ((rc = k16_ws_reserve(ctx, SL.ws_segoff, (size_t)(nb + 1) * 4))) return rc;
        if ((rc = k16_ws_reserve(ctx, SL.ws_sorted, (size_t)n * W * 4))) return rc;
        if ((rc = k16_ws_reserve(ctx, SL.ws_scan, (size_t)(2 * 4096 + 16) * 4))) return rc;
    }
    const uint32_t big_cap = nb;
    if (!reuse && (rc = k16_ws_reserve(ctx, SL.ws_big, ((size_t)2 * big_cap + GIANT_CAP) * 4))) return rc;
    uint32_t seg = MIN_SEG;
    {
        const uint64_t mean = (uint64_t)n * W / nb;
        if (mean >= 24) seg = (uint32_t)std::min<uint64_t>(256, (mean * 2 + 7) & ~7ull);
    }
    if (ctx->forced_seg) seg = ctx->forced_seg;
    if (ctx->tune.seg) seg = std::max(1, std::min((int)MAX_SEG, ctx->tune.seg));
    const size_t max_segs = (size_t)nb + (size_t)n * W / seg + 1;
    if (!reuse && (rc = k16_ws_reserve(ctx, SL.ws_segbucket, max_segs * 8 + 64))) return rc;

    uint32_t* zr = (uint32_t*)SL.ws_counts.p;
    SortArgs  a;
    a.d_scalars = d_scalars;
    a.n = n; a.c = c; a.W = W; a.flat = flat; a.nb = nb; a.seg = seg; a.big_cap = big_cap;
    a.max_segs = max_segs; a.zr_words = zr_words;
    a.zr         = zr;
    a.misc       = zr;
    a.gcount     = zr + 16;
    a.gcursor    = zr + 16 + GS;
    a.seg_hist   = zr + 16 + 2 * GS;
    a.counts     = zr + ZR_HDR;
    a.offsets    = (uint32_t*)SL.ws_offsets.p;
    a.cursor     = (uint32_t*)SL.ws_cursor.p;
    a.seg_off    = (uint32_t*)SL.ws_segoff.p;
    a.sorted     = (uint32_t*)SL.ws_sorted.p;
    a.scan_tmp   = (uint32_t*)SL.ws_scan.p;
    a.big_list   = (uint32_t*)SL.ws_big.p;
    a.seg_bucket = (uint32_t*)SL.ws_segbucket.p;
    a.seg_order  = a.seg_bucket + max_segs;
    a.conv_in    = conv_in;
    a.conv_out   = conv_out;
    a.remap      = nullptr;
    a.skip       = nullptr;
    a.hs[0] = a.hs[1] = a.hs[2] = nullptr;
    *out         = a;
    return K16_OK;
}

static bool msm_sort_is_plain_partition(const k16_ctx* ctx, uint64_t n, unsigned c, bool flat, const uint64_t* skip)
{
    if (flat || n > (1u << 24) || c < 4 || c > 16 || ctx->tune.atomic_sort) return false;
    const bool staged = !skip && n >= (1u << 16) && c == 16 && n < (1u << 24);
    return !staged;
}

int msm_sort_derive_launch(k16_ctx* ctx, hipStream_t st, const SortArgs& a, const k16_ctx::Lane& owner, const uint64_t* drop)
{
    const uint32_t*  gstart = (const uint32_t*)owner.ws_lvl_d.p;
    const uint32_t*  gslice = gstart + SORT_GS;
    const uint32_t*  part   = gstart + 2 * SORT_GS;
    k16_stat_scope   ss(ctx, "msm_sort", st);
    K16_HIP(ctx, hipMemsetAsync(a.zr, 0, a.zr_words * 4, st));
    constexpr unsigned SCAN_BLK = SCAN_T * SCAN_PER_DEFAULT;
    const unsigned     nblk     = (a.nb + SCAN_BLK - 1) / SCAN_BLK;
    if (nblk > 4096) {
        ctx->err = "msm: too many buckets for the scan workspace";
        return K16_ERR_ARG;
    }
    const unsigned sgrid_max = (unsigned)(((uint64_t)a.n * a.W) / PART_SLICE) + 1;
#define K16_DERIVE(CC)                                                                                                       \
    case CC: {                                                                                                               \
        typedef PartCfg<CC> CFG;                                                                                             \
        const unsigned      nb1 = CFG::NB1, sgrid = nb1 + sgrid_max;                                                         \
        hipLaunchKernelGGL((k_part_bins<CFG, 0>), dim3(sgrid), dim3(256), 0, st, gstart, gslice, nb1, part, a.counts, a.sorted, \
                           a.remap, (const uint8_t*)nullptr, 0u, drop);                                                      \
        hipLaunchKernelGGL(k_scan2_totals<SCAN_PER_DEFAULT>, dim3(nblk), dim3(SCAN_T), 0, st, a.counts, a.nb, a.seg, a.scan_tmp); \
        hipLaunchKernelGGL(k_scan2_apply<SCAN_PER_DEFAULT>, dim3(nblk), dim3(SCAN_T), 0, st, a.counts, a.nb, a.seg, a.scan_tmp, \
                           a.offsets, a.cursor, a.seg_off, a.misc, a.big_list, a.big_cap, a.big_list + a.big_cap,            \
                           a.big_list + a.big_cap + GIANT_CAP, a.seg_bucket, a.seg_hist);                                    \
        hipLaunchKernelGGL((k_part_bins<CFG, 1>), dim3(sgrid), dim3(256), 0, st, gstart, gslice, nb1, part, a.cursor, a.sorted, \
                           a.remap, (const uint8_t*)nullptr, 0u, drop);                                                      \
    } break;
    switch (a.c) {
        K16_DERIVE(4) K16_DERIVE(5) K16_DERIVE(6) K16_DERIVE(7) K16_DERIVE(8) K16_DERIVE(9) K16_DERIVE(10) K16_DERIVE(11)
        K16_DERIVE(12) K16_DERIVE(13) K16_DERIVE(14) K16_DERIVE(15) K16_DERIVE(16)
    default: ctx->err = "unsupported window size"; return K16_ERR_ARG;
    }
#undef K16_DERIVE
    const unsigned segrid = (unsigned)std::min<size_t>((a.max_segs + 256 * SEG_PER_THREAD - 1) / (256 * SEG_PER_THREAD), 1024);
    hipLaunchKernelGGL(k_seg_scatter, dim3(segrid), dim3(256), 0, st, a.offsets, a.seg_off, a.misc + 1, a.seg_bucket, a.seg_hist,
                       a.seg_hist + (MAX_SEG + 1), a.seg_order, a.seg);
    K16_HIP(ctx, hipGetLastError());
    return K16_OK;
}

template <class E>
int msm_enqueue_t(k16_ctx* ctx, const typename E::Row* d_bases, const void* d_scalars, uint64_t n, unsigned c,
                  bool flat = false, const void* conv_in = nullptr)
{
    void* conv_out = conv_in ? (void*)d_bases : nullptr;
    const unsigned W  = flat ? (257 + c - 1) / c : n_windows(c);
    const uint32_t nb = flat ? (1u << (c - 1)) : (W << (c - 1));
    if (flat && (uint64_t)n * W >= (1ull << 25)) {
        ctx->err = "fixed-base msm: n * windows must stay below 2^25";
        return K16_ERR_ARG;
    }
    k16_ctx::Lane& L  = ctx->lanes[ctx->cur_lane];
    hipStream_t    st = k16_lane_stream(ctx, ctx->cur_lane);

    int src_lane = (ctx->reuse_sort && ctx->reuse_sort_lane >= 0 && ctx->reuse_sort_lane < k16_ctx::N_LANES)
                       ? ctx->reuse_sort_lane : ctx->cur_lane;
    const uint64_t* acc_skip = ctx->acc_skip_next;
    ctx->acc_skip_next       = nullptr;
    const uint64_t* skip = ctx->skip_next;
    ctx->skip_next       = nullptr;
    const int derive_lane = ctx->derive_lane;
    ctx->derive_lane      = -1;
    bool derive = false, derive_fallback = false;
    if (derive_lane >= 0) {
        if (derive_lane >= k16_ctx::N_LANES || derive_lane == ctx->cur_lane || !skip || ctx->reuse_sort) {
            ctx->err = "msm: a derived bucket sort needs another lane's sort, a row mask, and no reuse request";
            return K16_ERR_ARG;
        }
        const k16_ctx::Lane& D = ctx->lanes[derive_lane];
        if (!(D.sorted_scalars == d_scalars && D.sorted_n == n && D.sorted_c == c)) {
            ctx->err = "msm: no matching bucket sort on the lane to derive from";
            return K16_ERR_ARG;
        }
        if (D.sorted_plain_partition && !flat) {
            derive = true;
        } else {
            derive_fallback = true;
            src_lane        = derive_lane;
            if (!acc_skip) acc_skip = skip;
        }
    }
    k16_ctx::Lane& SL  = ctx->lanes[src_lane];
#ifdef K16_LAB
    static const char* probe        = getenv("K16_LAB_PROBE");
    static const bool  probe_nosort = probe && strstr(probe, "nosort"), probe_notail = probe && strstr(probe, "notail");
    if (probe_nosort && L.sorted_scalars == d_scalars) ctx->reuse_sort = true;
#else
    constexpr bool probe_notail = false;
#endif
    const bool reuse   = derive_fallback || (ctx->reuse_sort && SL.sorted_scalars == d_scalars && SL.sorted_n == n &&
                                             SL.sorted_c == c && SL.sorted_skip == skip);
    ctx->reuse_sort      = false;
    ctx->reuse_sort_lane = -1;
    if (!reuse && &SL != &L) {
        ctx->err = "msm: no matching bucket sort on the lane to reuse";
        return K16_ERR_ARG;
    }

    int      rc;
    SortArgs sa;
    if ((rc = msm_sort_plan(ctx, SL, d_scalars, n, c, flat, reuse, conv_in, conv_out, &sa))) return rc;
    sa.remap        = ctx->remap_next;
    ctx->remap_next = nullptr;
    sa.skip         = skip;
    for (int k = 0; k < 3; k++) {
        sa.hs[k]        = ctx->hs_next[k];
        ctx->hs_next[k] = nullptr;
    }
    if (sa.hs[0] && (reuse || derive || !sa.hs[1] || !sa.hs[2])) {
        ctx->err = "msm: scalars still to be formed need a bucket sort of their own";
        return K16_ERR_ARG;
    }
    if (sa.remap && flat) {
        ctx->err = "msm: a fixed-base table cannot be combined with a row indirection";
        return K16_ERR_ARG;
    }
    const uint32_t seg = sa.seg, big_cap = sa.big_cap;
    const size_t   max_segs = sa.max_segs;
    uint32_t *misc = sa.misc, *offsets = sa.offsets, *seg_off = sa.seg_off, *sorted = sa.sorted, *big_list = sa.big_list,
             *seg_bucket = sa.seg_bucket, *seg_order = sa.seg_order;
    if ((rc = k16_ws_reserve(ctx, L.ws_lvl_c, (size_t)GIANT_CAP * GIANT_BLOCKS * sizeof(typename E::Pt)))) return rc;
    if ((rc = k16_ws_reserve(ctx, L.ws_partial, max_segs * sizeof(typename E::Pt)))) return rc;
    typename E::Pt*  partial   = (typename E::Pt*)L.ws_partial.p;

    const bool trace = ctx->tune.trace;
#define K16_TRACE_PT(msg)                                                             \
    if (trace) {                                                                      \
        hipError_t te_ = hipStreamSynchronize(st);                                    \
        fprintf(stderr, "[k16 trace] %s : %s\n", msg, hipGetErrorString(te_));       \
    }
    K16_TRACE_PT("enter");
    const bool tick_on = ctx->tune.trace_enq;
    struct Ticks {
        bool on;
        std::chrono::steady_clock::time_point t0, last;
        char buf[512];
        int  len = 0;
        void tick(const char* what)
        {
            if (!on) return;
            auto now = std::chrono::steady_clock::now();
            double ms = std::chrono::duration<double, std::milli>(now - last).count();
            last = now;
            if (ms > 0.3 && len < 440) len += snprintf(buf + len, sizeof buf - len, " %s=%.2f", what, ms);
        }
        ~Ticks()
        {
            if (on && len) fprintf(stderr, "[k16 enq]%s\n", buf);
        }
    } tk{tick_on, std::chrono::steady_clock::now(), std::chrono::steady_clock::now(), {0}};
    if (reuse && &SL != &L) K16_HIP(ctx, hipStreamWaitEvent(st, SL.sort_done, 0));
    const bool use_graphs = ctx->graphs_on && !trace;
    const bool sort_graphs = use_graphs && !sa.skip && !sa.remap && !skip && !derive;
    auto sort_body = [&]() -> int { return msm_sort_launch(ctx, L, st, sa, [&](const char* w) { tk.tick(w); }); };
    if (derive) {
        const k16_ctx::Lane& D = ctx->lanes[derive_lane];
        K16_HIP(ctx, hipStreamWaitEvent(st, D.sort_done, 0));
        auto derive_body = [&]() -> int { return msm_sort_derive_launch(ctx, st, sa, D, skip); };
        const k16_ctx::Lane::GraphKey key{-1 - derive_lane, d_scalars, n, c, seg, 0u, 0};
        rc = sort_graphs ? run_graph_section(ctx, L, st, key, derive_body) : derive_body();
        if (rc) return rc;
        L.sorted_scalars         = d_scalars;
        L.sorted_n               = n;
        L.sorted_c               = c;
        L.sorted_skip            = skip;
        L.sorted_plain_partition = false;
        K16_HIP(ctx, hipEventRecord(L.sort_done, st));
        K16_HIP(ctx, hipStreamWaitEvent(k16_lane_stream(ctx, derive_lane), L.sort_done, 0));
    } else if (!reuse) {
        const k16_ctx::Lane::GraphKey key{0, d_scalars, n, c, seg, flat ? 1u : 0u, sa.hs[0] ? 1 : 0};
        rc = sort_graphs ? run_graph_section(ctx, L, st, key, sort_body) : sort_body();
        if (rc) return rc;
        L.sorted_scalars         = d_scalars;
        L.sorted_n               = n;
        L.sorted_c               = c;
        L.sorted_skip            = skip;
        L.sorted_plain_partition = msm_sort_is_plain_partition(ctx, n, c, flat, skip);
        K16_HIP(ctx, hipEventRecord(L.sort_done, st));
    }
    tk.tick("sorted");
    K16_TRACE_PT("sorted");
    if (ctx->serialize_acc && ctx->last_acc_done && ctx->last_acc_done != L.acc_done)
        K16_HIP(ctx, hipStreamWaitEvent(st, ctx->last_acc_done, 0));
    {
        k16_stat_scope ss(ctx, "msm_accumulate", st);
        const unsigned grid = (unsigned)std::min<size_t>((max_segs + 127) / 128, 256 * 64);
        if (acc_skip)
            hipLaunchKernelGGL((k_accumulate_skip<E>), dim3(grid), dim3(128 * E::ALPP), 0, st, d_bases, sorted, offsets, seg_off,
                               seg_bucket, seg_order, misc + 1, partial, seg, acc_skip);
        else
            hipLaunchKernelGGL((k_accumulate<E>), dim3(grid), dim3(128 * E::ALPP), 0, st, d_bases, sorted, offsets, seg_off,
                               seg_bucket, seg_order, misc + 1, partial, seg);
    }
    if (ctx->serialize_acc) {
        K16_HIP(ctx, hipEventRecord(L.acc_done, st));
        ctx->last_acc_done = L.acc_done;
    }
    tk.tick("acc");
    K16_TRACE_PT("accumulated");
    const uint32_t Wr      = flat ? std::max<uint32_t>(1u, (1u << (c - 1)) >> 15) : W;
    const uint32_t win_mag = flat ? (1u << (c - 1)) / Wr : (1u << (c - 1));
    uint32_t mlog = std::min<uint32_t>(ctx->wsum_mlog_cap, WSUM_MLOG_MAX);
    while (mlog > 0 && (((uint64_t)Wr * win_mag) >> mlog) < 16384) mlog--;
    const uint32_t U     = win_mag >> mlog;
    uint32_t       nbits = 0;
    while ((1u << nbits) < U) nbits++;
    ctx->pend_mlog  = mlog;
    ctx->pend_nbits = nbits;
    ctx->pend_wr    = Wr;
    if ((size_t)Wr * (nbits + 2) * sizeof(typename E::Pt) > k16_ctx::NARROW_OFF) {
        ctx->err = "msm: pinned staging slot too small";
        return K16_ERR_ARG;
    }
    auto tail_body = [&]() -> int {
    if (probe_notail) return K16_OK;
    {
        k16_stat_scope ss(ctx, "msm_fold", st);
        typename E::Pt* giant_scratch = (typename E::Pt*)L.ws_lvl_c.p;
        const uint32_t  nS = std::min<uint32_t>((nb + 255) / 256, 4096), nT = 512, nB = 256;
        hipLaunchKernelGGL((k_fold_all<E>), dim3(nS + nT + nB + GIANT_BLOCKS), dim3(256 * E::LPP), 256 * sizeof(typename E::Pt), st,
                           seg_off, nb, big_list + big_cap + GIANT_CAP, big_list, big_list + big_cap, misc, big_cap, partial,
                           giant_scratch, nS, nT, nB);
        hipLaunchKernelGGL((k_fold_giant_b<E>), dim3(8), dim3(64 * E::LPP), 64 * sizeof(typename E::Pt), st, seg_off,
                           big_list + big_cap, misc + 3, partial, giant_scratch);
    }
    tk.tick("fold");
    K16_TRACE_PT("folded");
    {
        k16_stat_scope ss(ctx, "msm_reduce", st);
        size_t lb = (size_t)Wr * U * sizeof(typename E::Pt);
        if ((rc = k16_ws_reserve(ctx, L.ws_lvl_a, lb))) return rc;
        if ((rc = k16_ws_reserve(ctx, L.ws_lvl_b, lb))) return rc;
        typename E::Pt* S = (typename E::Pt*)L.ws_lvl_a.p;
        typename E::Pt* G = (typename E::Pt*)L.ws_lvl_b.p;
        typename E::Pt* T = (typename E::Pt*)((char*)ctx->pinned_dev + (size_t)ctx->enq_slot * k16_ctx::SLOT_BYTES);
        unsigned nthr = 2 * Wr * U;
        if (flat && sizeof(typename E::Pt) < 200)
            hipLaunchKernelGGL((k_wsum_level1<E, true>), dim3((nthr + 63) / 64), dim3(64 * E::LPP), 0, st, U, Wr, 1u << mlog, seg_off, c,
                               flat ? 1u : 0u, partial, S, G);
        else
            hipLaunchKernelGGL((k_wsum_level1<E>), dim3((nthr + 63) / 64), dim3(64 * E::LPP), 0, st, U, Wr, 1u << mlog, seg_off, c,
                               flat ? 1u : 0u, partial, S, G);
        hipLaunchKernelGGL((k_wsum_bits<E>), dim3(Wr * (nbits + 2)), dim3(256 * E::LPP), 256 * sizeof(typename E::Pt), st, S, G, U, nbits,
                           T);
        tk.tick("wsum");
    }
    tk.tick("d2h");
    K16_TRACE_PT("reduced");
    K16_HIP(ctx, hipGetLastError());
    return K16_OK;
    };
    {
        const k16_ctx::Lane::GraphKey key{1 + (int)sizeof(typename E::Pt), (const void*)&SL, n, c,
                                          seg * 64u + mlog, flat ? 1u : 0u, ctx->enq_slot};
        return use_graphs ? run_graph_section(ctx, L, st, key, tail_body) : tail_body();
    }
}

constexpr unsigned NARROW_BITS = k16_scalar_classes::BITS;

template <class E>
__global__ void __launch_bounds__(256) k_masked_sums(const typename E::Row* __restrict__ bases, const uint32_t* __restrict__ lists,
                                                     uint64_t cap_n, const uint32_t* __restrict__ cnt, uint32_t K,
                                                     typename E::Pt* __restrict__ partial, uint32_t* __restrict__ chunk_tab)
{
    k16_short_kernel_prio();
    extern __shared__ uint4 lds_raw[];
    typename E::Pt*         lds = reinterpret_cast<typename E::Pt*>(lds_raw);
    __shared__ uint32_t     pre[NARROW_BITS + 1], len[NARROW_BITS];
    const uint32_t          CH = 256u * K;
    if (threadIdx.x == 0) {
        uint32_t run = 0;
        for (unsigned b = 0; b < NARROW_BITS; b++) {
            pre[b] = run;
            len[b] = cnt[b];
            run += (len[b] + CH - 1) / CH;
        }
        pre[NARROW_BITS] = run;
    }
    k16_lds_sync();
    if (blockIdx.x == 0 && threadIdx.x <= NARROW_BITS) chunk_tab[threadIdx.x] = pre[threadIdx.x];
    for (uint32_t chunk = blockIdx.x; chunk < pre[NARROW_BITS]; chunk += gridDim.x) {
        unsigned b = 0;
        while (b + 1 < NARROW_BITS && pre[b + 1] <= chunk) b++;
        const uint32_t* __restrict__ list = lists + (size_t)b * cap_n;
        const uint32_t lo = (chunk - pre[b]) * CH, hi = min(lo + CH, len[b]);
        typename E::Pt acc = E::zero();
        uint32_t       j   = lo + threadIdx.x;
        if (j < hi) {
            typename E::AffR nxt = E::load_row(&bases[list[j]]);
            if constexpr (E::has_aff_add) {
                if (j + 256 < hi) {
                    typename E::AffR first = nxt, second = E::load_row(&bases[list[j + 256]]);
                    if (j + 512 < hi) nxt = E::load_row(&bases[list[j + 512]]);
                    acc = E::add_aff(first, second);
                    j += 512;
                }
            }
#pragma clang loop unroll(disable)
            for (; j < hi; j += 256) {
                typename E::AffR cur = nxt;
                if (j + 256 < hi) nxt = E::load_row(&bases[list[j + 256]]);
                acc = E::madd(acc, cur);
            }
        }
        lds[threadIdx.x] = acc;
        k16_lds_sync();
#pragma clang loop unroll(disable)
        for (unsigned o = 128; o > 0; o >>= 1) {
            if (threadIdx.x < o) {
                typename E::Pt a = lds[threadIdx.x], c = lds[threadIdx.x + o];
                lds[threadIdx.x] = E::add(a, c);
            }
            k16_lds_sync();
        }
        if (threadIdx.x == 0) store_vec(&partial[chunk], lds[0]);
        k16_lds_sync();
    }
}
template <class E>
__global__ void __launch_bounds__(256) k_masked_final(const typename E::Pt* __restrict__ partial, const uint32_t* __restrict__ chunk_tab,
                                                      typename E::Pt* __restrict__ out)
{
    k16_short_kernel_prio();
    extern __shared__ uint4 lds_raw[];
    typename E::Pt*         lds = reinterpret_cast<typename E::Pt*>(lds_raw);
    const uint32_t          lo = chunk_tab[blockIdx.x], hi = chunk_tab[blockIdx.x + 1];
    typename E::Pt          acc = E::zero();
#pragma clang loop unroll(disable)
    for (uint32_t j = lo + threadIdx.x; j < hi; j += 256) acc = E::add(acc, load_vec(&partial[j]));
    lds[threadIdx.x] = acc;
    k16_lds_sync();
#pragma clang loop unroll(disable)
    for (unsigned o = 128; o > 0; o >>= 1) {
        if (threadIdx.x < o && threadIdx.x + o < hi - lo) {
            typename E::Pt a = lds[threadIdx.x], c = lds[threadIdx.x + o];
            lds[threadIdx.x] = E::add(a, c);
// ... 46 lines not shown
```

keyless-zk-proofs_amd/k16.py:

```python
import ctypes as C
import os

import numpy as np

HERE = os.path.dirname(os.path.abspath(__file__))
LIB_PATH = os.environ.get("K16_LIB_PATH") or os.path.join(HERE, "libk16.so")

G1, G2 = 0, 1
OPT_PIPELINED_MSM = 1
OPT_GRAPHS = 2
OPT_SHARED_GPU = 3
OPT_YIELDING_WAITS = 4
FQ, FR = 0, 1
FQ9, FR9, FQ2N, FQ2H = 2, 3, 4, 5
G1_ENG9, G2_ENG2N, G2_PAIR = 2, 3, 4
OP_ADD, OP_SUB, OP_NEG, OP_MUL, OP_SQR, OP_TOMONT, OP_FROMMONT, OP_LAZY_ADDMUL, OP_LAZY_SUBMUL = range(9)
PT_ADD, PT_MADD, PT_DBL, PT_MADD_ACC = range(4)
AFF_BYTES = {G1: 64, G2: 128, G1_ENG9: 64, G2_ENG2N: 128, G2_PAIR: 128}
XYZZ_BYTES = {G1: 128, G2: 256, G1_ENG9: 128, G2_ENG2N: 256, G2_PAIR: 256}


def op_bound(op, ka=0, kb=0):
    return op | (ka << 8) | (kb << 12)

ERR = {0: "OK", -1: "NO_DEVICE", -2: "HIP", -3: "ARG", -4: "IO", -5: "FORMAT", -6: "CURVE", -7: "BUFFER", -8: "NOMEM"}

SYMBOLS = [
    "k16_runtime_hw_queues", "k16_device_count", "k16_host_threads", "k16_ctx_create", "k16_ctx_create_ex", "k16_ctx_destroy", "k16_last_error", "k16_sync", "k16_stream",
    "k16_dev_alloc", "k16_dev_free", "k16_h2d", "k16_d2h", "k16_host_register", "k16_host_unregister",
    "k16_timer_start", "k16_timer_stop", "k16_kernel_stats_enable", "k16_kernel_stats_reset", "k16_kernel_stats_get",
    "k16_ctx_set_option", "k16_msm", "k16_msm_host", "k16_msm_enqueue", "k16_msm_finish", "k16_msm_finish_group", "k16_msm_pending", "k16_msm_abort_all", "k16_msm_bases_prepare", "k16_msm_enqueue_prepared", "k16_msm_fixed_base_info", "k16_msm_fixed_base_prepare", "k16_msm_enqueue_fixed_base", "k16_msm_set_window_bits", "k16_msm_set_lane", "k16_points_sum",
    "k16_msm_zero_row_mask", "k16_msm_set_zero_row_mask", "k16_msm_sort_from_lane", "k16_scalar_classes_create", "k16_scalar_classes_destroy", "k16_scalar_classes_build", "k16_scalar_classes_counts", "k16_msm_enqueue_classified",
    "k16_ntt", "k16_ntt_host", "k16_synth_points", "k16_synth_points_scalars", "k16_field_op_vec", "k16_point_op_vec", "k16_coop_exec",
    "k16_prover_create", "k16_prover_create_mem", "k16_prover_create_shared", "k16_prover_destroy", "k16_prover_info",
    "k16_prover_prove_file", "k16_prover_prove_file_timed", "k16_prover_prove_mem", "k16_prover_compact_buffers", "k16_prover_prove_compact", "k16_fullprover_prove_mem", "k16_fullprover_compact_lease", "k16_fullprover_prove_compact", "k16_fullprover_compact_cancel", "k16_prover_last_h", "k16_prover_warmup_status",
    "k16_vk_create", "k16_vk_destroy", "k16_verify_batch", "k16_verify_coop_gt", "k16_pairing_vec",
    "k16_points_check", "k16_verify_batch_checked", "k16_zkey_check", "k16_zkey_check_file",
    "k16_verify_batch_folded", "k16_verify_fold_gt",
    "k16_vk_create_from_zkey", "k16_vk_create_from_zkey_file", "k16_prover_set_vk", "k16_prover_prove_mem_verified",
    "k16_prover_prove_compact_verified", "k16_prover_prove_file_verified", "k16_verify_split_gt", "k16_fullprover_set_verify",
    "k16_r1cs_create", "k16_r1cs_create_mem", "k16_r1cs_destroy", "k16_r1cs_info", "k16_r1cs_check_mem", "k16_r1cs_check_file",
    "k16_r1cs_check_prover_witness", "k16_r1cs_last_values", "k16_r1cs_match_zkey",
    "k16_r1cs_unbound_wires", "k16_r1cs_wire_constraints", "k16_r1cs_incidences", "k16_r1cs_second_values",
    "k16_r1cs_determined_wires", "k16_r1cs_complete_witness", "k16_r1cs_complete_witness_ex", "k16_r1cs_boolean_wires",
    "k16_r1cs_determined_wires_ex", "k16_r1cs_held_wires", "k16_r1cs_open_system", "k16_r1cs_open_direction",
    "k16_r1cs_open_system_ex", "k16_r1cs_open_direction_ex",
    "k16_prover_set_r1cs", "k16_prover_last_check", "k16_fullprover_set_r1cs", "k16_fullprover_last_rejection",
    "k16_r1cs_setup_size", "k16_r1cs_setup", "k16_r1cs_setup_file", "k16_generator_mul", "k16_generator_mul_info",
    "k16_msm_sharded_create", "k16_msm_sharded_destroy", "k16_msm_sharded_count", "k16_msm_sharded_range", "k16_msm_sharded_ctx",
    "k16_msm_sharded_last_error", "k16_msm_sharded_set_bases", "k16_msm_sharded_set_bases_device", "k16_msm_sharded_run",
    "k16_msm_sharded_run_device", "k16_msm_sharded_set_piece_rows", "k16_msm_sharded_last_ms",
    "k16_rank_comm_unique_id", "k16_rank_comm_load_error", "k16_rank_comm_create", "k16_rank_comm_destroy", "k16_rank_comm_allgather_fold", "k16_rank_comm_allgather_start", "k16_rank_comm_allgather_finish",
]

_lib = None


class K16Error(RuntimeError):
    def __init__(self, rc, msg=""):
        super().__init__("k16 error %s (%d) %s" % (ERR.get(rc, "?"), rc, msg))
        self.rc = rc


def load():
    global _lib
    if _lib is not None:
        return _lib
    if not os.path.exists(LIB_PATH):
        raise K16Error(-1, "libk16.so not built: run `python -c 'import __graft_entry__ as g; g.build()'`")
    L = C.CDLL(LIB_PATH)
    vp, u64, i32, u32, sz = C.c_void_p, C.c_uint64, C.c_int, C.c_uint32, C.c_size_t
    L.k16_runtime_hw_queues.argtypes = [i32]
    L.k16_ctx_create.argtypes = [i32, C.POINTER(vp)]
    L.k16_ctx_create_ex.argtypes = [i32, i32, C.POINTER(vp)]
    L.k16_ctx_destroy.argtypes = [vp]
    L.k16_ctx_destroy.restype = None
    L.k16_last_error.argtypes = [vp]
    L.k16_last_error.restype = C.c_char_p
    L.k16_sync.argtypes = [vp]
    L.k16_stream.argtypes = [vp]
    L.k16_stream.restype = vp
    L.k16_dev_alloc.argtypes = [vp, sz, C.POINTER(vp)]
    L.k16_dev_free.argtypes = [vp, vp]
    L.k16_h2d.argtypes = [vp, vp, vp, sz]
    L.k16_d2h.argtypes = [vp, vp, vp, sz]
    L.k16_host_register.argtypes = [vp, vp, sz]
    L.k16_host_unregister.argtypes = [vp, vp]
    L.k16_timer_start.argtypes = [vp]
    L.k16_timer_stop.argtypes = [vp, C.POINTER(C.c_float)]
    L.k16_kernel_stats_enable.argtypes = [vp, i32]
    L.k16_kernel_stats_reset.argtypes = [vp]
    L.k16_kernel_stats_get.argtypes = [vp, C.c_char_p, C.POINTER(u64), C.POINTER(C.c_double)]
    L.k16_ctx_set_option.argtypes = [vp, i32, i32]
    L.k16_msm.argtypes = [vp, i32, vp, vp, u64, vp, vp]
    L.k16_msm_host.argtypes = [vp, i32, vp, vp, u64, vp, vp]
    L.k16_msm_enqueue.argtypes = [vp, i32, vp, vp, u64]
    L.k16_msm_finish.argtypes = [vp, vp, vp]
    L.k16_msm_finish_group.argtypes = [vp, i32, vp, vp]
    L.k16_msm_pending.argtypes = [vp]
    L.k16_msm_abort_all.argtypes = [vp]
    L.k16_msm_bases_prepare.argtypes = [vp, i32, vp, u64, vp]
    L.k16_msm_enqueue_prepared.argtypes = [vp, i32, vp, vp, u64]
    L.k16_msm_fixed_base_info.argtypes = [u64, C.POINTER(u32), C.POINTER(u64)]
    L.k16_msm_fixed_base_prepare.argtypes = [vp, i32, vp, u64, vp]
    L.k16_msm_enqueue_fixed_base.argtypes = [vp, i32, vp, vp, u64]
    L.k16_msm_set_window_bits.argtypes = [vp, u32]
    L.k16_msm_set_lane.argtypes = [vp, i32]
    L.k16_points_sum.argtypes = [i32, vp, u64, vp, vp]
    L.k16_msm_zero_row_mask.argtypes = [vp, i32, vp, u64, vp]
    L.k16_msm_set_zero_row_mask.argtypes = [vp, vp]
    L.k16_msm_sort_from_lane.argtypes = [vp, i32, i32]
    L.k16_scalar_classes_create.argtypes = [vp, u64, i32, C.POINTER(vp)]
    L.k16_scalar_classes_destroy.argtypes = [vp]
    L.k16_scalar_classes_destroy.restype = None
    L.k16_scalar_classes_build.argtypes = [vp, vp, vp, u64, C.POINTER(vp), i32, C.c_int64]
    L.k16_scalar_classes_counts.argtypes = [vp, vp, vp]
    L.k16_msm_enqueue_classified.argtypes = [vp, i32, vp, vp, i32]
    L.k16_ntt.argtypes = [vp, vp, u64, u64, i32]
    L.k16_ntt_host.argtypes = [vp, vp, u64, u64, i32]
    L.k16_synth_points.argtypes = [vp, i32, u64, u64, vp]
    L.k16_synth_points_scalars.argtypes = [vp, i32, vp, u64, vp]
    L.k16_field_op_vec.argtypes = [vp, i32, i32, vp, vp, vp, u64]
    L.k16_point_op_vec.argtypes = [vp, i32, i32, vp, vp, vp, u64]
    L.k16_coop_exec.argtypes = [vp, vp, u64, vp, vp, u64, C.c_uint32, C.c_uint32, vp, vp, vp, u64, vp]
    L.k16_prover_create.argtypes = [vp, C.c_char_p, C.POINTER(vp)]
    L.k16_prover_create_mem.argtypes = [vp, vp, sz, C.POINTER(vp)]
    L.k16_prover_create_shared.argtypes = [vp, vp, C.POINTER(vp)]
    L.k16_prover_destroy.argtypes = [vp]
    L.k16_prover_destroy.restype = None
    L.k16_prover_info.argtypes = [vp, C.POINTER(u32), C.POINTER(u32), C.POINTER(u32), C.POINTER(u64)]
    L.k16_prover_prove_file.argtypes = [vp, C.c_char_p, vp, vp, C.c_char_p, sz, C.POINTER(C.c_float)]
    L.k16_prover_prove_file_timed.argtypes = [vp, C.c_char_p, vp, vp, C.c_char_p, sz, C.POINTER(C.c_float), C.POINTER(C.c_float)]
    L.k16_prover_prove_mem.argtypes = [vp, vp, u64, vp, vp, C.c_char_p, sz, C.POINTER(C.c_float)]
    L.k16_prover_compact_buffers.argtypes = [vp, C.POINTER(vp), C.POINTER(vp), C.POINTER(vp), C.POINTER(u64)]
    L.k16_prover_prove_compact.argtypes = [vp, u64, vp, vp, C.c_char_p, sz, C.POINTER(C.c_float)]
    L.k16_prover_last_h.argtypes = [vp, vp]
    L.k16_fullprover_prove_mem.argtypes = [vp, vp, u64, C.c_char_p, sz, C.POINTER(i32)]
    L.k16_fullprover_compact_lease.argtypes = [vp, C.POINTER(vp), C.POINTER(vp), C.POINTER(vp), C.POINTER(vp), C.POINTER(u64), C.POINTER(u32)]
    L.k16_fullprover_prove_compact.argtypes = [vp, vp, u64, C.c_char_p, sz, C.POINTER(i32)]
    L.k16_fullprover_compact_cancel.argtypes = [vp, vp]
    L.k16_prover_warmup_status.argtypes = [vp]
    L.k16_vk_create.argtypes = [vp, vp, vp, vp, vp, vp, u32, C.POINTER(vp)]
    L.k16_vk_destroy.argtypes = [vp]
    L.k16_vk_destroy.restype = None
    L.k16_verify_batch.argtypes = [vp, vp, vp, vp, u64, vp]
    L.k16_verify_coop_gt.argtypes = [vp, vp, vp, vp, u64, vp]
    L.k16_pairing_vec.argtypes = [vp, vp, vp, u64, vp]
    L.k16_points_check.argtypes = [vp, i32, vp, u64, vp]
    L.k16_verify_batch_checked.argtypes = [vp, vp, vp, vp, u64, vp, vp]
    L.k16_verify_batch_folded.argtypes = [vp, vp, vp, vp, u64, vp, vp, C.POINTER(C.c_uint8)]
    L.k16_verify_fold_gt.argtypes = [vp, vp, vp, vp, u64, vp, vp]
    L.k16_vk_create_from_zkey.argtypes = [vp, vp, sz, C.POINTER(vp)]
    L.k16_vk_create_from_zkey_file.argtypes = [vp, C.c_char_p, C.POINTER(vp)]
    L.k16_prover_set_vk.argtypes = [vp, vp]
    L.k16_prover_prove_mem_verified.argtypes = [vp, vp, u64, vp, vp, C.c_char_p, sz, C.POINTER(C.c_float), vp, C.POINTER(C.c_uint8)]
    L.k16_prover_prove_compact_verified.argtypes = [vp, u64, vp, vp, C.c_char_p, sz, C.POINTER(C.c_float), vp, C.POINTER(C.c_uint8)]
    L.k16_prover_prove_file_verified.argtypes = [vp, C.c_char_p, vp, vp, C.c_char_p, sz, C.POINTER(C.c_float), C.POINTER(C.c_float), vp, C.POINTER(C.c_uint8)]
    L.k16_fullprover_set_verify.argtypes = [vp, i32]
    L.k16_verify_split_gt.argtypes = [vp, vp, vp, vp, u64, vp, vp]
    L.k16_zkey_check.argtypes = [vp, vp, sz, C.POINTER(u32), C.POINTER(u64), C.POINTER(C.c_uint8), C.POINTER(u64)]
    L.k16_zkey_check_file.argtypes = [vp, C.c_char_p, C.POINTER(u32), C.POINTER(u64), C.POINTER(C.c_uint8), C.POINTER(u64)]
    L.k16_r1cs_create.argtypes = [vp, C.c_char_p, C.POINTER(vp)]
    L.k16_r1cs_create_mem.argtypes = [vp, vp, sz, C.POINTER(vp)]
    L.k16_r1cs_destroy.argtypes = [vp]
    L.k16_r1cs_destroy.restype = None
    L.k16_r1cs_info.argtypes = [vp, C.POINTER(u32), C.POINTER(u32), C.POINTER(u32), C.POINTER(u64)]
    L.k16_r1cs_check_mem.argtypes = [vp, vp, vp, u64, C.POINTER(u64), vp, u32]
    L.k16_r1cs_check_file.argtypes = [vp, vp, C.c_char_p, C.POINTER(u64), vp, u32]
    L.k16_r1cs_check_prover_witness.argtypes = [vp, vp, C.POINTER(u64), vp, u32]
    L.k16_r1cs_last_values.argtypes = [vp, u32, vp]
    L.k16_r1cs_match_zkey.argtypes = [vp, vp, vp, sz, C.POINTER(u32)]
    L.k16_r1cs_unbound_wires.argtypes = [vp, C.POINTER(u64), C.POINTER(u64), vp, vp, u32, vp]
    L.k16_r1cs_wire_constraints.argtypes = [vp, u32, C.POINTER(u64), vp, u32]
    L.k16_r1cs_incidences.argtypes = [vp, C.POINTER(u64)]
    L.k16_r1cs_second_values.argtypes = [vp, C.POINTER(u64), vp, vp, u32, vp]
    L.k16_r1cs_determined_wires.argtypes = [vp, vp, u32, C.POINTER(u64), C.POINTER(u64), C.POINTER(u64), C.POINTER(u32), vp, u32,
                                            vp, vp, vp]
    L.k16_r1cs_complete_witness.argtypes = [vp, vp, vp, u32, C.POINTER(u64), C.POINTER(u64), C.POINTER(u64), C.POINTER(u32),
                                            C.POINTER(u64), vp, u32, C.POINTER(u64), vp, u32, vp, vp, vp]
    L.k16_r1cs_complete_witness_ex.argtypes = [vp, vp, vp, u32, u32, C.POINTER(u64), C.POINTER(u64), C.POINTER(u64), C.POINTER(u32),
                                               C.POINTER(u64), vp, u32, C.POINTER(u64), vp, u32, vp, vp, vp, C.POINTER(u64),
                                               C.POINTER(u64), vp, u32, vp]
    L.k16_r1cs_boolean_wires.argtypes = [vp, C.POINTER(u64), vp]
    L.k16_r1cs_determined_wires_ex.argtypes = [vp, vp, u32, u32, C.POINTER(u64), C.POINTER(u64), C.POINTER(u64), C.POINTER(u32), vp, u32,
                                               vp, vp, vp, C.POINTER(u64), vp]
    L.k16_r1cs_held_wires.argtypes = [vp, C.POINTER(u64), vp]
    L.k16_r1cs_open_system.argtypes = [vp, vp] + [C.POINTER(u64)] * 7 + [vp, vp, u32, vp, vp]
    L.k16_r1cs_open_direction.argtypes = [vp, vp, u32, C.POINTER(C.c_uint8)] + [C.POINTER(u32)] * 4 + [C.POINTER(u64), vp, vp, u32]
    L.k16_r1cs_open_system_ex.argtypes = [vp, vp, u32] + [C.POINTER(u64)] * 7 + [vp, vp, u32, vp, vp]
# ... 53 lines not shown
    def upload(self, arr):
        arr = np.ascontiguousarray(arr)
        assert arr.nbytes <= self.nbytes
        self.ctx._chk(self.ctx.L.k16_h2d(self.ctx.h, self.ptr, _p(arr), arr.nbytes))
        return self

    def download(self, dtype=np.uint8, shape=None):
        out = np.empty(self.nbytes, dtype=np.uint8)
        self.ctx._chk(self.ctx.L.k16_d2h(self.ctx.h, _p(out), self.ptr, self.nbytes))
        out = out.view(dtype)
        return out.reshape(shape) if shape is not None else out

    def free(self):
        if self.ptr:
            self.ctx.L.k16_dev_free(self.ctx.h, self.ptr)
            self.ptr = None


class Context:
    def __init__(self, device=0, stream_offset=0):
        self.L = load()
        h = C.c_void_p()
        rc = self.L.k16_ctx_create_ex(device, stream_offset, C.byref(h)) if stream_offset else self.L.k16_ctx_create(device, C.byref(h))
        if rc:
            raise K16Error(rc, "k16_ctx_create(device=%d): no usable HIP device" % device)
        self.h = h
        self.device = device

    def close(self):
        if self.h:
            if not getattr(self, "borrowed", False):
                self.L.k16_ctx_destroy(self.h)
            self.h = None

    def _chk(self, rc):
        if rc:
            raise K16Error(rc, (self.L.k16_last_error(self.h) or b"").decode())

    def sync(self):
        self._chk(self.L.k16_sync(self.h))

    def alloc(self, nbytes):
        return DeviceBuffer(self, nbytes)

    def to_device(self, arr):
        arr = np.ascontiguousarray(arr)
        return DeviceBuffer(self, max(arr.nbytes, 16)).upload(arr)

    def host_register(self, arr):
        assert arr.flags["C_CONTIGUOUS"]
        self._chk(self.L.k16_host_register(self.h, arr.ctypes.data_as(C.c_void_p), arr.nbytes))

    def host_unregister(self, arr):
        self._chk(self.L.k16_host_unregister(self.h, arr.ctypes.data_as(C.c_void_p)))

    def timer_start(self):
        self._chk(self.L.k16_timer_start(self.h))

    def timer_stop(self):
        ms = C.c_float()
        self._chk(self.L.k16_timer_stop(self.h, C.byref(ms)))
        return ms.value

    def stats_enable(self, on=True):
        self._chk(self.L.k16_kernel_stats_enable(self.h, int(on)))

    def stats_reset(self):
        self._chk(self.L.k16_kernel_stats_reset(self.h))

    def stats_get(self, name):
        n, ms = C.c_uint64(), C.c_double()
        self._chk(self.L.k16_kernel_stats_get(self.h, name.encode(), C.byref(n), C.byref(ms)))
        return n.value, ms.value

    def set_option(self, option, value):
        self._chk(self.L.k16_ctx_set_option(self.h, option, value))

    def set_lane(self, lane):
        self._chk(self.L.k16_msm_set_lane(self.h, lane))

    def set_window_bits(self, c):
        self._chk(self.L.k16_msm_set_window_bits(self.h, c))

    def msm_device(self, group, d_bases, d_scalars, n):
        x = np.zeros(XYZZ_BYTES[group], dtype=np.uint8)
        a = np.zeros(AFF_BYTES[group], dtype=np.uint8)
        self._chk(self.L.k16_msm(self.h, group, d_bases.ptr if d_bases else None,
                                 d_scalars.ptr if d_scalars else None, n, _p(x), _p(a)))
        return x.tobytes(), a.tobytes()

    def msm_enqueue(self, group, d_bases, d_scalars, n):
        self._chk(self.L.k16_msm_enqueue(self.h, group, d_bases.ptr, d_scalars.ptr, n))

    def bases_prepare(self, group, d_bases, n):
        out = self.alloc(max(n * AFF_BYTES[group], 16))
        self._chk(self.L.k16_msm_bases_prepare(self.h, group, d_bases.ptr, n, out.ptr))
        self.sync()
        return out

    def msm_enqueue_prepared(self, group, d_prepared, d_scalars, n):
        self._chk(self.L.k16_msm_enqueue_prepared(self.h, group, d_prepared.ptr, d_scalars.ptr, n))

    def fixed_base_prepare(self, group, d_bases, n):
        c, rows = C.c_uint32(0), C.c_uint64(0)
        self._chk(self.L.k16_msm_fixed_base_info(n, C.byref(c), C.byref(rows)))
        if c.value == 0:
            return None, 0
        out = self.alloc(rows.value * AFF_BYTES[group])
        self._chk(self.L.k16_msm_fixed_base_prepare(self.h, group, d_bases.ptr, n, out.ptr))
        self.sync()
        return out, c.value

    def msm_enqueue_fixed_base(self, group, d_table, d_scalars, n):
        self._chk(self.L.k16_msm_enqueue_fixed_base(self.h, group, d_table.ptr, d_scalars.ptr, n))

    def zero_row_mask(self, group, d_rows, n):
        d = self.alloc(max((n + 63) // 64 * 8, 16))
        self._chk(self.L.k16_msm_zero_row_mask(self.h, group, d_rows.ptr, n, d.ptr))
        self.sync()
        return d

    def msm_set_zero_row_mask(self, d_mask):
        self._chk(self.L.k16_msm_set_zero_row_mask(self.h, d_mask.ptr if d_mask is not None else None))

    def msm_sort_from_lane(self, lane, derive=False):
        self._chk(self.L.k16_msm_sort_from_lane(self.h, lane, 1 if derive else 0))

    def classes_create(self, max_n, max_sets=1):
        h = C.c_void_p()
        self._chk(self.L.k16_scalar_classes_create(self.h, max_n, max_sets, C.byref(h)))
        return h

    def classes_destroy(self, cls):
        self.L.k16_scalar_classes_destroy(cls)

    def classes_build(self, cls, d_scalars, n, masks=None, n_wide_bound=-1):
        masks = masks if masks is not None else [None]
        arr = (C.c_void_p * len(masks))(*[(m.ptr if m is not None else None) for m in masks])
        self._chk(self.L.k16_scalar_classes_build(self.h, cls, d_scalars.ptr if d_scalars else None, n, arr, len(masks), n_wide_bound))

    def classes_counts(self, cls, n_sets):
        out = np.zeros(n_sets * 8 + 1, dtype=np.uint32)
        self._chk(self.L.k16_scalar_classes_counts(self.h, cls, _p(out)))
        return out

    def msm_enqueue_classified(self, group, d_prepared, cls, set_index=0):
        self._chk(self.L.k16_msm_enqueue_classified(self.h, group, d_prepared.ptr if d_prepared else None, cls, set_index))

    def msm_finish(self, group):
        x = np.zeros(XYZZ_BYTES[group], dtype=np.uint8)
        a = np.zeros(AFF_BYTES[group], dtype=np.uint8)
        self._chk(self.L.k16_msm_finish_group(self.h, group, _p(x), _p(a)))
        return x.tobytes(), a.tobytes()

    def msm_pending(self):
        return self.L.k16_msm_pending(self.h)

    def msm_abort_all(self):
        self._chk(self.L.k16_msm_abort_all(self.h))

    def msm(self, group, bases, scalars):
        bases = np.ascontiguousarray(bases, dtype=np.uint8)
        scalars = np.ascontiguousarray(scalars, dtype=np.uint8)
        n = scalars.shape[0] if scalars.ndim == 2 else 0
        x = np.zeros(XYZZ_BYTES[group], dtype=np.uint8)
        a = np.zeros(AFF_BYTES[group], dtype=np.uint8)
# ... 804 lines not shown
```

Before: 785.6 million points/s.

## Add GLV endomorphism path for G1 MSM with split scalars and doubled rows

Adds a GLV scalar decomposition for BN254 G1. Each 254-bit scalar becomes two signed half-size scalars, and the converting counting pass emits the beta-multiplied endomorphism rows next to the converted bases. The Pippenger window count drops to about 126/c+1 windows per half while the number of entries per point doubles. This roughly halves the bucket-reduction and window-combination work. In exchange it costs extra decomposition arithmetic, twice the converted-base storage, and sort reuse is disabled on this path.

```diff
diff --git a/include/k16.h b/include/k16.h
--- a/include/k16.h
+++ b/include/k16.h
@@ -88,6 +88,7 @@
 #define K16_MSM_LANES 4
 int k16_msm_set_lane(k16_ctx* ctx, int lane);
 int k16_msm_set_window_bits(k16_ctx* ctx, unsigned c);
+int k16_msm_uses_endomorphism(k16_ctx* ctx, int group, uint64_t n, uint64_t* n_min, uint64_t* n_max);
 
 typedef struct k16_msm_shards k16_msm_shards;
 int         k16_msm_sharded_create(const int* devices, int n_devices, int group, uint64_t n, k16_msm_shards** out);
diff --git a/keyless-zk-proofs_amd/csrc/bn254_glv.h b/keyless-zk-proofs_amd/csrc/bn254_glv.h
--- /dev/null
+++ b/keyless-zk-proofs_amd/csrc/bn254_glv.h
@@ -0,0 +1,140 @@
+#pragma once
+#include <stdint.h>
+
+#ifndef K16_HD
+#define K16_HD inline
+#endif
+
+namespace k16 {
+
+struct GlvC {
+    static constexpr uint32_t R[8] = {0xf0000001u, 0x43e1f593u, 0x79b97091u, 0x2833e848u,
+                                      0x8181585du, 0xb85045b6u, 0xe131a029u, 0x30644e72u};
+    static constexpr uint32_t LAMBDA[8] = {0xb99c90ddu, 0x8b17ea66u, 0x8d8daaa7u, 0x5bfc4108u, 0x41a91758u, 0xb3c4d79du, 0u, 0u};
+    static constexpr uint32_t BETA9[9] = {0x0a337995u, 0x158d1d23u, 0x189c9b98u, 0x12fa4e45u, 0x185faadcu,
+                                          0x0176f16du, 0x0eed93bau, 0x14291140u, 0x000c0afeu};
+    static constexpr uint32_t N[2]  = {0x94d213e3u, 0x89d32568u};
+    static constexpr uint32_t M1[4] = {0x7d4f1128u, 0x8211bbebu, 0xeeb859fcu, 0x6f4d8248u};
+    static constexpr uint32_t M2[4] = {0x1221250bu, 0x0be4e154u, 0xeeb859fdu, 0x6f4d8248u};
+    static constexpr unsigned SHIFT_WORDS = 9;
+    static constexpr uint32_t G1[4] = {0x6eb9c714u, 0xc7e0b3d7u, 0xd91d232eu, 0x00000002u};
+    static constexpr uint32_t G2[6] = {0xa5e38cfbu, 0x391eb18du, 0x7a7bd9d4u, 0xa773d2cfu, 0x4ccef014u, 0x00000002u};
+};
+
+struct GlvSplit {
+    uint32_t k1[4], k2[4];
+    uint32_t neg1, neg2;
+};
+
+template <int G>
+K16_HD void glv_mulhi_round(const uint32_t (&k)[8], const uint32_t (&g)[G], uint32_t (&d)[4])
+{
+    constexpr int TW = 8 + G > (int)GlvC::SHIFT_WORDS + 4 ? 8 + G : (int)GlvC::SHIFT_WORDS + 4;
+    uint32_t      t[TW];
+#pragma unroll
+    for (int i = 0; i < TW; i++) t[i] = 0;
+#pragma unroll
+    for (int i = 0; i < 8; i++) {
+        uint64_t carry = 0;
+#pragma unroll
+        for (int j = 0; j < G; j++) {
+            const uint64_t acc = (uint64_t)k[i] * g[j] + t[i + j] + carry;
+            t[i + j]           = (uint32_t)acc;
+            carry              = acc >> 32;
+        }
+        t[i + G] = (uint32_t)carry;
+    }
+    uint64_t c = 0x80000000ull;
+#pragma unroll
+    for (int i = GlvC::SHIFT_WORDS - 1; i < 8 + G; i++) {
+        c += t[i];
+        t[i] = (uint32_t)c;
+        c >>= 32;
+    }
+#pragma unroll
+    for (int i = 0; i < 4; i++) d[i] = t[GlvC::SHIFT_WORDS + i];
+}
+
+template <int NB>
+K16_HD void glv_mullo128(const uint32_t (&a)[4], const uint32_t (&b)[NB], uint32_t (&o)[4])
+{
+#pragma unroll
+    for (int i = 0; i < 4; i++) o[i] = 0;
+#pragma unroll
+    for (int i = 0; i < 4; i++) {
+        uint64_t carry = 0;
+#pragma unroll
+        for (int j = 0; j < NB; j++) {
+            if (i + j >= 4) continue;
+            const uint64_t acc = (uint64_t)a[i] * b[j] + o[i + j] + carry;
+            o[i + j]           = (uint32_t)acc;
+            carry              = acc >> 32;
+        }
+        if (i + NB < 4) o[i + NB] = (uint32_t)carry;
+    }
+}
+K16_HD void glv_sub128(uint32_t (&a)[4], const uint32_t (&b)[4])
+{
+    int64_t c = 0;
+#pragma unroll
+    for (int i = 0; i < 4; i++) {
+        c += (int64_t)a[i] - (int64_t)b[i];
+        a[i] = (uint32_t)c;
+        c >>= 32;
+    }
+}
+K16_HD uint32_t glv_abs128(uint32_t (&a)[4])
+{
+    const uint32_t neg = a[3] >> 31;
+    if (neg) {
+        uint64_t c = 1;
+#pragma unroll
+        for (int i = 0; i < 4; i++) {
+            c += (uint32_t)~a[i];
+            a[i] = (uint32_t)c;
+            c >>= 32;
+        }
+    }
+    return neg;
+}
+
+K16_HD GlvSplit glv_split(const uint32_t (&kin)[8])
+{
+    uint32_t k[8];
+#pragma unroll
+    for (int i = 0; i < 8; i++) k[i] = kin[i];
+#pragma unroll
+    for (int rep = 0; rep < 5; rep++) {
+        uint32_t d[8];
+        int64_t  c = 0;
+#pragma unroll
+        for (int i = 0; i < 8; i++) {
+            c += (int64_t)k[i] - (int64_t)GlvC::R[i];
+            d[i] = (uint32_t)c;
+            c >>= 32;
+        }
+        if (c == 0) {
+#pragma unroll
+            for (int i = 0; i < 8; i++) k[i] = d[i];
+        }
+    }
+    uint32_t d1[4], d2[4];
+    glv_mulhi_round<4>(k, GlvC::G1, d1);
+    glv_mulhi_round<6>(k, GlvC::G2, d2);
+    GlvSplit s;
+    uint32_t t[4];
+#pragma unroll
+    for (int i = 0; i < 4; i++) s.k1[i] = k[i];
+    glv_mullo128<2>(d1, GlvC::N, t);
+    glv_sub128(s.k1, t);
+    glv_mullo128<4>(d2, GlvC::M2, t);
+    glv_sub128(s.k1, t);
+    glv_mullo128<4>(d1, GlvC::M1, s.k2);
+    glv_mullo128<2>(d2, GlvC::N, t);
+    glv_sub128(s.k2, t);
+    s.neg1 = glv_abs128(s.k1);
+    s.neg2 = glv_abs128(s.k2);
+    return s;
+}
+
+}
diff --git a/keyless-zk-proofs_amd/csrc/ctx.h b/keyless-zk-proofs_amd/csrc/ctx.h
--- a/keyless-zk-proofs_amd/csrc/ctx.h
+++ b/keyless-zk-proofs_amd/csrc/ctx.h
@@ -68,7 +68,7 @@
     struct Lane {
         hipStream_t stream = nullptr;
         k16_devbuf  ws_counts, ws_offsets, ws_cursor, ws_sorted, ws_segoff, ws_segbucket, ws_partial, ws_big,
-            ws_lvl_a, ws_lvl_b, ws_lvl_c, ws_lvl_d, ws_scan, ws_conv, ws_narrow;
+            ws_lvl_a, ws_lvl_b, ws_lvl_c, ws_lvl_d, ws_scan, ws_conv, ws_narrow, ws_glv;
         struct GraphEntry {
             int            state = 0;
             hipGraphExec_t exec  = nullptr;
@@ -126,6 +126,7 @@
     const uint64_t* skip_next = nullptr;
     const uint64_t* acc_skip_next = nullptr;
     int             derive_lane   = -1;
+    bool            chunked_msm   = false;
     unsigned        ntt_wg_per_cu = 4;
     const void*     hs_next[3]    = {nullptr, nullptr, nullptr};
     bool        serialize_acc = false;
diff --git a/keyless-zk-proofs_amd/csrc/ctx.hip b/keyless-zk-proofs_amd/csrc/ctx.hip
--- a/keyless-zk-proofs_amd/csrc/ctx.hip
+++ b/keyless-zk-proofs_amd/csrc/ctx.hip
@@ -123,7 +123,7 @@
     for (auto& L : c->lanes) {
         k16_devbuf* bufs[] = {&L.ws_counts, &L.ws_offsets, &L.ws_cursor, &L.ws_sorted, &L.ws_segoff, &L.ws_segbucket,
                               &L.ws_partial, &L.ws_big, &L.ws_lvl_a, &L.ws_lvl_b, &L.ws_lvl_c,
-                              &L.ws_lvl_d, &L.ws_scan, &L.ws_conv, &L.ws_narrow};
+                              &L.ws_lvl_d, &L.ws_scan, &L.ws_conv, &L.ws_narrow, &L.ws_glv};
         for (auto* b : bufs)
             if (b->p) (void)hipFree(b->p);
     }
diff --git a/keyless-zk-proofs_amd/csrc/msm_api.hip b/keyless-zk-proofs_amd/csrc/msm_api.hip
--- a/keyless-zk-proofs_amd/csrc/msm_api.hip
+++ b/keyless-zk-proofs_amd/csrc/msm_api.hip
@@ -17,6 +17,8 @@
 int k16_msm_enqueue_fixed_g1(k16_ctx* ctx, const void* d_table, const void* d_scalars, uint64_t n, unsigned c);
 int k16_msm_enqueue_classified_g1(k16_ctx* ctx, const void* d_rows, const k16_scalar_classes* cls, int set, unsigned c, bool* has_wide, int phase);
 int k16_msm_enqueue_classified_g2(k16_ctx* ctx, const void* d_rows, const k16_scalar_classes* cls, int set, unsigned c, bool* has_wide, int phase);
+bool k16_msm_glv_ok_g1(const k16_ctx* ctx, uint64_t n, unsigned c);
+void k16_msm_glv_range_g1(uint64_t* n_min, uint64_t* n_max);
 
 namespace {
 constexpr unsigned MAX_C = 16;
@@ -287,6 +289,7 @@
         rc = group == K16_G1 ? k16_msm_enqueue_g1(ctx, d_bases, d_scalars, n, c, prepared)
                              : k16_msm_enqueue_g2(ctx, d_bases, d_scalars, n, c, prepared);
         if (rc) return rc;
+        pd.w     = ctx->pend_wr;
         pd.nbits = ctx->pend_nbits;
         pd.mlog  = ctx->pend_mlog;
         K16_HIP(ctx, hipEventRecord(ctx->pend_ev[idx], k16_lane_stream(ctx, ctx->cur_lane)));
@@ -297,6 +300,18 @@
         ctx->pend_count++;
     }
     return K16_OK;
+}
+
+extern "C" int k16_msm_uses_endomorphism(k16_ctx* ctx, int group, uint64_t n, uint64_t* n_min, uint64_t* n_max)
+{
+    return k16_guard(ctx, [&]() -> int {
+    if (!ctx || (group != K16_G1 && group != K16_G2)) return K16_ERR_ARG;
+    uint64_t lo, hi;
+    k16_msm_glv_range_g1(&lo, &hi);
+    if (n_min) *n_min = lo;
+    if (n_max) *n_max = hi;
+    return group == K16_G1 && n != 0 && n < (1ull << 32) / 80 && k16_msm_glv_ok_g1(ctx, n, choose_c(ctx, n)) ? 1 : 0;
+    });
 }
 
 extern "C" int k16_msm_enqueue(k16_ctx* ctx, int group, const void* d_bases, const void* d_scalars, uint64_t n)
@@ -580,12 +595,14 @@
         enq++;
         return k16_msm_enqueue(ctx, group, (const char*)d_bases + lo * pb, (const char*)d_scalars + lo * 32, cnt);
     };
+    ctx->chunked_msm = true;
     rc = enqueue_next();
     while (!rc && fin < chunks) {
         if (enq < chunks) rc = enqueue_next();
         if (!rc) rc = k16_msm_finish(ctx, parts.data() + (size_t)fin * xb, nullptr);
         fin++;
     }
+    ctx->chunked_msm = false;
     ctx->cur_lane = saved;
     if (rc) {
         (void)k16_msm_abort_all(ctx);
diff --git a/keyless-zk-proofs_amd/csrc/msm_g1.hip b/keyless-zk-proofs_amd/csrc/msm_g1.hip
--- a/keyless-zk-proofs_amd/csrc/msm_g1.hip
+++ b/keyless-zk-proofs_amd/csrc/msm_g1.hip
@@ -11,22 +11,38 @@
     K16_HIP(ctx, hipGetLastError());
     return K16_OK;
 }
+static bool msm_fuse_convert_ok(const k16_ctx* ctx, uint64_t n)
+{
+    return n <= (1u << 24) && !ctx->reuse_sort && ctx->derive_lane < 0 && !ctx->graphs_on && !ctx->tune.atomic_sort;
+}
+constexpr uint64_t GLV_N_MIN = 1ull << 12, GLV_N_MAX = 1ull << 23;
+bool k16_msm_glv_ok_g1(const k16_ctx* ctx, uint64_t n, unsigned c)
+{
+    return msm_fuse_convert_ok(ctx, n) && n >= GLV_N_MIN && n <= GLV_N_MAX && c >= 8 && c <= 16 && !ctx->chunked_msm && !ctx->skip_next &&
+           !ctx->acc_skip_next && !ctx->remap_next && !ctx->hs_next[0];
+}
+void k16_msm_glv_range_g1(uint64_t* n_min, uint64_t* n_max)
+{
+    *n_min = GLV_N_MIN;
+    *n_max = GLV_N_MAX;
+}
 int k16_msm_enqueue_g1(k16_ctx* ctx, const void* d_bases, const void* d_scalars, uint64_t n, unsigned c, int prepared)
 {
     const k16::G1Aff* rows = (const k16::G1Aff*)d_bases;
     const void*       conv_in = nullptr;
+    bool              glv = false;
     if (!prepared) {
         k16_ctx::Lane& L = ctx->lanes[ctx->cur_lane];
-        int rc = k16_ws_reserve(ctx, L.ws_conv, (size_t)n * sizeof(k16::G1Aff));
+        glv = k16_msm_glv_ok_g1(ctx, n, c);
+        int rc = k16_ws_reserve(ctx, L.ws_conv, (size_t)(glv ? 2 * n : n) * sizeof(k16::G1Aff));
         if (rc) return rc;
         rows = (const k16::G1Aff*)L.ws_conv.p;
-        const bool fuse = n <= (1u << 24) && !ctx->reuse_sort && ctx->derive_lane < 0 && !ctx->graphs_on && !ctx->tune.atomic_sort;
-        if (fuse)
+        if (msm_fuse_convert_ok(ctx, n))
             conv_in = d_bases;
         else if ((rc = k16_msm_prepare_g1(ctx, d_bases, n, L.ws_conv.p, k16_lane_stream(ctx, ctx->cur_lane))))
             return rc;
     }
-    return msm_enqueue_t<Eng9>(ctx, rows, d_scalars, n, c, false, conv_in);
+    return msm_enqueue_t<Eng9>(ctx, rows, d_scalars, n, c, false, conv_in, glv);
 }
 
 namespace {
diff --git a/keyless-zk-proofs_amd/csrc/msm_kernels.inc b/keyless-zk-proofs_amd/csrc/msm_kernels.inc
--- a/keyless-zk-proofs_amd/csrc/msm_kernels.inc
+++ b/keyless-zk-proofs_amd/csrc/msm_kernels.inc
@@ -5,6 +5,7 @@
 #include "ctx.h"
 #include "bn254_fq2pair.h"
 #include "bn254_fq9.h"
+#include "bn254_glv.h"
 
 using namespace k16;
 
@@ -18,6 +19,7 @@
 constexpr unsigned MIN_C     = 4;
 
 __host__ __device__ inline unsigned n_windows(unsigned c) { return (256 + c - 1) / c + 1; }
+__host__ __device__ inline unsigned n_windows_glv(unsigned c) { return 126 / c + 1; }
 
 __device__ __forceinline__ void k16_lds_sync()
 {
@@ -93,6 +95,30 @@
         carry              = neg;
         const uint32_t m   = neg ? FULL - v : v;
         if (m) f(w, m - 1u, neg);
+    }
+}
+
+template <unsigned C, class Fn>
+__device__ __forceinline__ void for_signed_digits_glv(const uint32_t (&k)[8], Fn f)
+{
+    constexpr unsigned W    = 126 / C + 1;
+    constexpr uint32_t HALF = 1u << (C - 1), FULL = 1u << C;
+#pragma unroll
+    for (unsigned h = 0; h < 2; h++) {
+        const uint32_t s[4] = {k[4 * h], k[4 * h + 1], k[4 * h + 2], k[4 * h + 3] & 0x7fffffffu};
+        const uint32_t sgn  = k[4 * h + 3] >> 31;
+        uint32_t       carry = 0;
+#pragma unroll
+        for (unsigned w = 0; w < W; w++) {
+            const unsigned bit = w * C, wd = bit >> 5, sh = bit & 31;
+            uint64_t       x   = s[wd];
+            if (wd + 1 < 4) x |= (uint64_t)s[wd + 1] << 32;
+            const uint32_t v   = ((uint32_t)(x >> sh) & (FULL - 1u)) + carry;
+            const uint32_t neg = v > HALF ? 1u : 0u;
+            carry              = neg;
+            const uint32_t m   = neg ? FULL - v : v;
+            if (m) f(w, m - 1u, neg ^ sgn, h);
+        }
     }
 }
 
@@ -154,6 +180,23 @@
     static constexpr unsigned NB1 = W << HI;
     static constexpr unsigned SHIFT = 24;
     static constexpr bool     FLAT  = false;
+    static constexpr bool     GLV   = false;
+    static constexpr unsigned EPP   = W;
+    static constexpr unsigned TILE  = PART_TILE;
+};
+template <unsigned CC>
+struct PartCfgGlv {
+    static constexpr unsigned C   = CC;
+    static constexpr unsigned W   = 126 / C + 1;
+    static constexpr unsigned BB  = C - 1;
+    static constexpr unsigned LO  = BB > 7 ? 7 : BB;
+    static constexpr unsigned LO4 = LO;
+    static constexpr unsigned HI  = BB - LO;
+    static constexpr unsigned NB1 = W << HI;
+    static constexpr unsigned SHIFT = 24;
+    static constexpr bool     FLAT  = false;
+    static constexpr bool     GLV   = true;
+    static constexpr unsigned EPP   = 2 * W;
     static constexpr unsigned TILE  = PART_TILE;
 };
 template <unsigned CC>
@@ -167,6 +210,8 @@
     static constexpr unsigned NB1 = 1u << HI;
     static constexpr unsigned SHIFT = 25;
     static constexpr bool     FLAT  = true;
+    static constexpr bool     GLV   = false;
+    static constexpr unsigned EPP   = W;
     static constexpr unsigned TILE  = PART_TILE;
 };
 
@@ -231,9 +276,10 @@
                                               uint32_t* __restrict__ gstart, uint32_t* __restrict__ gslice,
                                               const uint64_t* __restrict__ skip = nullptr,
                                               const k16::Fr* __restrict__ hs_a = nullptr, const k16::Fr* __restrict__ hs_b = nullptr,
-                                              const k16::Fr* __restrict__ hs_c = nullptr)
+                                              const k16::Fr* __restrict__ hs_c = nullptr, uint4* __restrict__ glv_out = nullptr)
 {
     static_assert(!HS || (!SCATTER && !CONV), "the H scalars are formed by the plain counting pass");
+    static_assert(!P::GLV || SCATTER || CONV, "the endomorphism rows are made by the converting counting pass");
     k16_short_kernel_prio();
     extern __shared__ uint32_t  part_lds[];
     __shared__ uint32_t         sh[256];
@@ -249,10 +295,12 @@
     const uint32_t              ntiles = (uint32_t)((n + P::TILE - 1) / P::TILE);
     auto bin_of = [](unsigned w, uint32_t m1) -> uint32_t { return P::FLAT ? (m1 >> P::LO) : ((w << P::HI) + (m1 >> P::LO)); };
     auto digits = [](const uint32_t (&k)[8], auto f) {
-        if constexpr (P::FLAT)
-            for_signed_digits_flat<P::C>(k, f);
+        if constexpr (P::GLV)
+            for_signed_digits_glv<P::C>(k, f);
+        else if constexpr (P::FLAT)
+            for_signed_digits_flat<P::C>(k, [&](unsigned w, uint32_t m1, uint32_t neg) { f(w, m1, neg, 0u); });
         else
-            for_signed_digits<P::C>(k, f);
+            for_signed_digits<P::C>(k, [&](unsigned w, uint32_t m1, uint32_t neg) { f(w, m1, neg, 0u); });
     };
     if (SCATTER) {
         if (blockIdx.x == 0) {
@@ -287,7 +335,7 @@
 #pragma unroll
         for (unsigned p = 0; p < PPT; p++) {
             uint32_t k[8] = {sc[p][0].x, sc[p][0].y, sc[p][0].z, sc[p][0].w, sc[p][1].x, sc[p][1].y, sc[p][1].z, sc[p][1].w};
-            digits(k, [&](unsigned w, uint32_t m1, uint32_t) { (void)hadd(bin_of(w, m1)); });
+            digits(k, [&](unsigned w, uint32_t m1, uint32_t, uint32_t) { (void)hadd(bin_of(w, m1)); });
         }
         k16_lds_sync();
         uint32_t got[BPT];
@@ -309,10 +357,10 @@
         for (unsigned p = 0; p < PPT; p++) {
             const uint64_t i = (uint64_t)tile * P::TILE + p * 256 + threadIdx.x;
             uint32_t k[8] = {sc[p][0].x, sc[p][0].y, sc[p][0].z, sc[p][0].w, sc[p][1].x, sc[p][1].y, sc[p][1].z, sc[p][1].w};
-            digits(k, [&](unsigned w, uint32_t m1, uint32_t neg) {
+            digits(k, [&](unsigned w, uint32_t m1, uint32_t neg, uint32_t half) {
                 uint32_t b   = bin_of(w, m1);
                 uint32_t r   = hadd(b);
-                uint32_t row = P::FLAT ? (uint32_t)(w * n + i) : (uint32_t)i;
+                uint32_t row = P::FLAT ? (uint32_t)(w * n + i) : (uint32_t)(i + half * n);
                 part[base[b] + r] = (neg << 31) | ((m1 & ((1u << P::LO) - 1u)) << P::SHIFT) | row;
             });
         }
@@ -337,8 +385,20 @@
                 hi = scalars[2 * i + 1];
             }
             uint32_t k[8] = {lo.x, lo.y, lo.z, lo.w, hi.x, hi.y, hi.z, hi.w};
+            if constexpr (P::GLV) {
+                const k16::GlvSplit s = k16::glv_split(k);
+#pragma unroll
+                for (unsigned q = 0; q < 4; q++) {
+                    k[q]     = s.k1[q];
+                    k[4 + q] = s.k2[q];
+                }
+                k[3] |= s.neg1 << 31;
+                k[7] |= s.neg2 << 31;
+                glv_out[2 * i]     = make_uint4(k[0], k[1], k[2], k[3]);
+                glv_out[2 * i + 1] = make_uint4(k[4], k[5], k[6], k[7]);
+            }
             if (!(skip && ((skip[i >> 6] >> (i & 63u)) & 1ull)))
-                digits(k, [&](unsigned w, uint32_t m1, uint32_t) { (void)hadd(bin_of(w, m1)); });
+                digits(k, [&](unsigned w, uint32_t m1, uint32_t, uint32_t) { (void)hadd(bin_of(w, m1)); });
             if constexpr (CONV) {
                 k16::Aff<k16::Fq> a = load_vec(&conv_in[i]);
                 k16::Aff9         c9 = k16::aff9_from_canonical(a);
@@ -346,6 +406,13 @@
                 k16::fq9_pack(o.x.v, c9.x);
                 k16::fq9_pack(o.y.v, c9.y);
                 store_vec(&conv_out[i], o);
+                if constexpr (P::GLV) {
+                    k16::Fq9 beta;
+#pragma unroll
+                    for (int q = 0; q < 9; q++) beta.l[q] = k16::GlvC::BETA9[q];
+                    k16::fq9_pack(o.x.v, k16::fmul9(c9.x, beta));
+                    store_vec(&conv_out[n + i], o);
+                }
             }
         }
         k16_lds_sync();
@@ -409,6 +476,8 @@
     static constexpr unsigned NB1 = 1u << HI;
     static constexpr unsigned SHIFT = 25;
     static constexpr bool     FLAT  = true;
+    static constexpr bool     GLV   = false;
+    static constexpr unsigned EPP   = W;
     static constexpr unsigned TILE  = PART_TILE;
 #ifndef K16_ST_TILE_FLAT
 #define K16_ST_TILE_FLAT 2048
@@ -426,13 +495,31 @@
     static constexpr unsigned NB1 = W << HI;
     static constexpr unsigned SHIFT = 24;
     static constexpr bool     FLAT  = false;
+    static constexpr bool     GLV   = false;
+    static constexpr unsigned EPP   = W;
+    static constexpr unsigned TILE  = PART_TILE;
+    static constexpr unsigned ST_TILE = 1024;
+};
+template <unsigned CC>
+struct PartCfgGlv5 {
+    static constexpr unsigned C   = CC;
+    static constexpr unsigned W   = 126 / C + 1;
+    static constexpr unsigned BB  = C - 1;
+    static constexpr unsigned LO  = BB > 8 ? 8 : BB;
+    static constexpr unsigned LO4 = 7;
+    static constexpr unsigned HI  = BB - LO;
+    static constexpr unsigned NB1 = W << HI;
+    static constexpr unsigned SHIFT = 24;
+    static constexpr bool     FLAT  = false;
+    static constexpr bool     GLV   = true;
+    static constexpr unsigned EPP   = 2 * W;
     static constexpr unsigned TILE  = PART_TILE;
     static constexpr unsigned ST_TILE = 1024;
 };
 constexpr unsigned ST_THREADS = 1024;
 template <class P>
 struct StageGeom {
-    static constexpr unsigned CAP       = P::ST_TILE * P::W;
+    static constexpr unsigned CAP       = P::ST_TILE * P::EPP;
     static constexpr unsigned NBP       = (P::NB1 + ST_THREADS - 1) / ST_THREADS;
     static constexpr unsigned LDS_BYTES = (3 * P::NB1 + 1 + ST_THREADS + CAP) * 4 + ((CAP + 3) & ~3u);
 };
@@ -453,10 +540,12 @@
     constexpr unsigned PPT = P::ST_TILE / ST_THREADS;
     auto bin_of = [](unsigned w, uint32_t m1) -> uint32_t { return P::FLAT ? (m1 >> P::LO) : ((w << P::HI) + (m1 >> P::LO)); };
     auto digits = [](const uint32_t (&k)[8], auto f) {
-        if constexpr (P::FLAT)
-            for_signed_digits_flat<P::C>(k, f);
+        if constexpr (P::GLV)
+            for_signed_digits_glv<P::C>(k, f);
+        else if constexpr (P::FLAT)
+            for_signed_digits_flat<P::C>(k, [&](unsigned w, uint32_t m1, uint32_t neg) { f(w, m1, neg, 0u); });
         else
-            for_signed_digits<P::C>(k, f);
+            for_signed_digits<P::C>(k, [&](unsigned w, uint32_t m1, uint32_t neg) { f(w, m1, neg, 0u); });
     };
     const uint32_t tile = blockIdx.x;
     uint4          sc[PPT][2];
@@ -475,7 +564,7 @@
 #pragma unroll
     for (unsigned p = 0; p < PPT; p++) {
         uint32_t k[8] = {sc[p][0].x, sc[p][0].y, sc[p][0].z, sc[p][0].w, sc[p][1].x, sc[p][1].y, sc[p][1].z, sc[p][1].w};
-        digits(k, [&](unsigned w, uint32_t m1, uint32_t) { atomicAdd(&cur[bin_of(w, m1)], 1u); });
+        digits(k, [&](unsigned w, uint32_t m1, uint32_t, uint32_t) { atomicAdd(&cur[bin_of(w, m1)], 1u); });
     }
     k16_lds_sync();
     {
@@ -518,9 +607,9 @@
     for (unsigned p = 0; p < PPT; p++) {
         const uint64_t i = (uint64_t)tile * P::ST_TILE + p * ST_THREADS + threadIdx.x;
         uint32_t k[8] = {sc[p][0].x, sc[p][0].y, sc[p][0].z, sc[p][0].w, sc[p][1].x, sc[p][1].y, sc[p][1].z, sc[p][1].w};
-        digits(k, [&](unsigned w, uint32_t m1, uint32_t neg) {
+        digits(k, [&](unsigned w, uint32_t m1, uint32_t neg, uint32_t half) {
             const uint32_t pos = atomicAdd(&cur[bin_of(w, m1)], 1u);
-            const uint32_t row = P::FLAT ? (uint32_t)(w * n + i) : (uint32_t)i;
+            const uint32_t row = P::FLAT ? (uint32_t)(w * n + i) : (uint32_t)(i + half * n);
             const uint32_t lo  = m1 & ((1u << P::LO) - 1u);
             st4[pos] = (neg << 31) | ((lo & ((1u << P::LO4) - 1u)) << P::SHIFT) | row;
             st1[pos] = (uint8_t)(lo >> P::LO4);
@@ -1559,6 +1648,9 @@
     const uint32_t* remap;
     const uint64_t* skip;
     const void*     hs[3];
+    bool     glv;
+    void*    glv_rec;
+    unsigned epp;
 };
 constexpr size_t SORT_GS = 8208;
 
@@ -1568,7 +1660,7 @@
     int            rc;
     const void*    d_scalars = a.d_scalars;
     const uint64_t n = a.n;
-    const unsigned c = a.c, W = a.W;
+    const unsigned c = a.c, W = a.epp;
     const bool     flat = a.flat;
     const uint32_t nb = a.nb, seg = a.seg, big_cap = a.big_cap;
     const size_t   max_segs = a.max_segs, zr_words = a.zr_words;
@@ -1587,6 +1679,10 @@
         K16_HIP(ctx, hipMemsetAsync(zr, 0, zr_words * 4, st));
         tick("memset");
         const bool staged = use_part && !skip && n >= (1u << 16) && ((flat && c == 20) || (!flat && c == 16 && n < (1u << 24)));
+        if (a.glv && (!use_part || !conv_in || flat || skip || remap || a.hs[0] || 2 * n > (1u << 24))) {
+            ctx->err = "msm: the endomorphism path was chosen for an MSM it does not serve";
+            return K16_ERR_ARG;
+        }
         const bool hs_fused = a.hs[0] && staged && flat && !a.conv_in;
         if (a.hs[0] && !hs_fused)
             hipLaunchKernelGGL(k_hs_fill, dim3((unsigned)((n + 255) / 256)), dim3(256), 0, st, (uint4*)const_cast<void*>(d_scalars), n,
@@ -1681,7 +1777,66 @@
         hipLaunchKernelGGL((k_part_bins<CFG, 1>), dim3(sgrid), dim3(256), 0, st, gstart, gslice, nb1, part, cursor, sorted,     \
                            remap, (const uint8_t*)part1, BS_CAP);                                                \
     }
-            if (staged && flat) {
+#define K16_PART_GLV(CC)                                                                                          \
+    case CC: {                                                                                                   \
+        typedef PartCfgGlv<CC> CFG;                                                                              \
+        const unsigned nb1   = CFG::NB1;                                                                         \
+        const unsigned ntiles = (unsigned)((n + CFG::TILE - 1) / CFG::TILE);                                     \
+        const unsigned pgrid  = std::min<unsigned>(ntiles, 256 * 4);                                             \
+        const unsigned sgrid = nb1 + (unsigned)(((uint64_t)n * W) / PART_SLICE) + 1;                              \
+        static_assert(CFG::NB1 + 1 <= GS, "partition tables too small");                                         \
+        hipLaunchKernelGGL((k_part<CFG, false, true>), dim3(pgrid), dim3(256), ((nb1 + 1) / 2 + nb1) * 4, st,     \
+                           (const uint4*)d_scalars, n, gcount, part, (const k16::Aff<k16::Fq>*)conv_in,            \
+                           (k16::Aff<k16::Fq>*)conv_out, (const uint32_t*)nullptr, (uint32_t*)nullptr,             \
+                           (uint32_t*)nullptr, (const uint64_t*)nullptr, (const k16::Fr*)nullptr,                  \
+                           (const k16::Fr*)nullptr, (const k16::Fr*)nullptr, (uint4*)a.glv_rec);                   \
+        hipLaunchKernelGGL((k_part<CFG, true>), dim3(ntiles), dim3(256), ((nb1 + 1) / 2 + nb1) * 4, st, (const uint4*)a.glv_rec, n, \
+                           gcursor, part, (const k16::Aff<k16::Fq>*)nullptr, (k16::Aff<k16::Fq>*)nullptr,         \
+                           (const uint32_t*)gcount, gstart, gslice, (const uint64_t*)nullptr);                    \
+        hipLaunchKernelGGL((k_part_bins<CFG, 0>), dim3(sgrid), dim3(256), 0, st, gstart, gslice, nb1, part, counts, sorted, remap); \
+        scans();                                                                                                 \
+        hipLaunchKernelGGL((k_part_bins<CFG, 1>), dim3(sgrid), dim3(256), 0, st, gstart, gslice, nb1, part, cursor, sorted, remap); \
+    } break;
+            if (a.glv && staged) {
+                typedef PartCfgGlv5<16> CFG;
+                const unsigned nb1    = CFG::NB1;
+                const unsigned ntiles = (unsigned)((n + CFG::TILE - 1) / CFG::TILE);
+                const unsigned pgrid  = std::min<unsigned>(ntiles, 256 * 4);
+                const unsigned sgrid  = nb1 + (unsigned)(((uint64_t)n * W) / PART_SLICE) + 1;
+                const unsigned stiles = (unsigned)((n + CFG::ST_TILE - 1) / CFG::ST_TILE);
+                const unsigned slds   = StageGeom<CFG>::LDS_BYTES;
+                const unsigned blds   = ((1u << CFG::LO) + BS_THREADS + BS_CAP) * 4;
+                static_assert(CFG::NB1 + 1 <= GS, "partition tables too small");
+                static_assert(StageGeom<CFG>::LDS_BYTES <= 160 * 1024, "stage does not fit the LDS");
+                static bool glv_attr = false;
+                if (!glv_attr) {
+                    K16_HIP(ctx, hipFuncSetAttribute((const void*)k_part_stage<CFG>, hipFuncAttributeMaxDynamicSharedMemorySize, (int)slds));
+                    K16_HIP(ctx, hipFuncSetAttribute((const void*)k_bins_stage<CFG>, hipFuncAttributeMaxDynamicSharedMemorySize, (int)blds));
+                    glv_attr = true;
+                }
+                uint8_t* part1 = (uint8_t*)(part + (size_t)n * W);
+                hipLaunchKernelGGL((k_part<CFG, false, true>), dim3(pgrid), dim3(256), ((nb1 + 1) / 2 + nb1) * 4, st,
+                                   (const uint4*)d_scalars, n, gcount, part, (const k16::Aff<k16::Fq>*)conv_in,
+                                   (k16::Aff<k16::Fq>*)conv_out, (const uint32_t*)nullptr, (uint32_t*)nullptr, (uint32_t*)nullptr,
+                                   (const uint64_t*)nullptr, (const k16::Fr*)nullptr, (const k16::Fr*)nullptr,
+                                   (const k16::Fr*)nullptr, (uint4*)a.glv_rec);
+                hipLaunchKernelGGL(k_bin_starts, dim3(1), dim3(WC_THREADS), 0, st, (const uint32_t*)gcount, nb1, gstart, gslice);
+                hipLaunchKernelGGL((k_part_stage<CFG>), dim3(stiles), dim3(ST_THREADS), slds, st, (const uint4*)a.glv_rec, n, gcursor,
+                                   part, part1, (const uint32_t*)gstart);
+                hipLaunchKernelGGL((k_bins_stage<CFG>), dim3(nb1), dim3(BS_THREADS), blds, st, (const uint32_t*)gstart, nb1,
+                                   (const uint32_t*)part, (const uint8_t*)part1, counts, sorted, remap);
+                hipLaunchKernelGGL((k_part_bins<CFG, 0>), dim3(sgrid), dim3(256), 0, st, gstart, gslice, nb1, part, counts, sorted,
+                                   remap, (const uint8_t*)part1, BS_CAP);
+                scans();
+                hipLaunchKernelGGL((k_part_bins<CFG, 1>), dim3(sgrid), dim3(256), 0, st, gstart, gslice, nb1, part, cursor, sorted,
+                                   remap, (const uint8_t*)part1, BS_CAP);
+            } else if (a.glv) {
+                switch (c) {
+                    K16_PART_GLV(8) K16_PART_GLV(9) K16_PART_GLV(10) K16_PART_GLV(11) K16_PART_GLV(12) K16_PART_GLV(13)
+                    K16_PART_GLV(14) K16_PART_GLV(15) K16_PART_GLV(16)
+                default: ctx->err = "unsupported window size for the endomorphism path"; return K16_ERR_ARG;
+                }
+            } else if (staged && flat) {
                 K16_PART_STAGED(PartCfgFlat5<20>)
             } else if (staged) {
                 K16_PART_STAGED(PartCfg5<16>)
@@ -1724,10 +1879,11 @@
 }
 
 int msm_sort_plan(k16_ctx* ctx, k16_ctx::Lane& SL, const void* d_scalars, uint64_t n, unsigned c, bool flat, bool reuse,
-                  const void* conv_in, void* conv_out, SortArgs* out)
+                  const void* conv_in, void* conv_out, SortArgs* out, bool glv = false)
 {
     int            rc;
-    const unsigned W  = flat ? (257 + c - 1) / c : n_windows(c);
+    const unsigned W  = flat ? (257 + c - 1) / c : glv ? n_windows_glv(c) : n_windows(c);
+    const unsigned epp = glv ? 2 * W : W;
     const uint32_t nb = flat ? (1u << (c - 1)) : (W << (c - 1));
     constexpr size_t GS     = SORT_GS;
     constexpr size_t ZR_HDR = (16 + 2 * GS + 2 * (MAX_SEG + 1) + 3) & ~(size_t)3;
@@ -1737,19 +1893,19 @@
         if ((rc = k16_ws_reserve(ctx, SL.ws_offsets, (size_t)(nb + 1) * 4))) return rc;
         if ((rc = k16_ws_reserve(ctx, SL.ws_cursor, (size_t)(nb + 1) * 4))) return rc;
         if ((rc = k16_ws_reserve(ctx, SL.ws_segoff, (size_t)(nb + 1) * 4))) return rc;
-        if ((rc = k16_ws_reserve(ctx, SL.ws_sorted, (size_t)n * W * 4))) return rc;
+        if ((rc = k16_ws_reserve(ctx, SL.ws_sorted, (size_t)n * epp * 4))) return rc;
         if ((rc = k16_ws_reserve(ctx, SL.ws_scan, (size_t)(2 * 4096 + 16) * 4))) return rc;
     }
     const uint32_t big_cap = nb;
     if (!reuse && (rc = k16_ws_reserve(ctx, SL.ws_big, ((size_t)2 * big_cap + GIANT_CAP) * 4))) return rc;
     uint32_t seg = MIN_SEG;
     {
-        const uint64_t mean = (uint64_t)n * W / nb;
+        const uint64_t mean = (uint64_t)n * epp / nb;
         if (mean >= 24) seg = (uint32_t)std::min<uint64_t>(256, (mean * 2 + 7) & ~7ull);
     }
     if (ctx->forced_seg) seg = ctx->forced_seg;
     if (ctx->tune.seg) seg = std::max(1, std::min((int)MAX_SEG, ctx->tune.seg));
-    const size_t max_segs = (size_t)nb + (size_t)n * W / seg + 1;
+    const size_t max_segs = (size_t)nb + (size_t)n * epp / seg + 1;
     if (!reuse && (rc = k16_ws_reserve(ctx, SL.ws_segbucket, max_segs * 8 + 64))) return rc;
 
     uint32_t* zr = (uint32_t*)SL.ws_counts.p;
@@ -1776,6 +1932,13 @@
     a.remap      = nullptr;
     a.skip       = nullptr;
     a.hs[0] = a.hs[1] = a.hs[2] = nullptr;
+    a.glv        = glv;
+    a.glv_rec    = nullptr;
+    a.epp        = epp;
+    if (glv) {
+        if ((rc = k16_ws_reserve(ctx, SL.ws_glv, (size_t)n * 32))) return rc;
+        a.glv_rec = SL.ws_glv.p;
+    }
     *out         = a;
     return K16_OK;
 }
@@ -1829,10 +1992,10 @@
 
 template <class E>
 int msm_enqueue_t(k16_ctx* ctx, const typename E::Row* d_bases, const void* d_scalars, uint64_t n, unsigned c,
-                  bool flat = false, const void* conv_in = nullptr)
+                  bool flat = false, const void* conv_in = nullptr, bool glv = false)
 {
     void* conv_out = conv_in ? (void*)d_bases : nullptr;
-    const unsigned W  = flat ? (257 + c - 1) / c : n_windows(c);
+    const unsigned W  = flat ? (257 + c - 1) / c : glv ? n_windows_glv(c) : n_windows(c);
     const uint32_t nb = flat ? (1u << (c - 1)) : (W << (c - 1));
     if (flat && (uint64_t)n * W >= (1ull << 25)) {
         ctx->err = "fixed-base msm: n * windows must stay below 2^25";
@@ -1887,7 +2050,11 @@
 
     int      rc;
     SortArgs sa;
-    if ((rc = msm_sort_plan(ctx, SL, d_scalars, n, c, flat, reuse, conv_in, conv_out, &sa))) return rc;
+    if (glv && (reuse || derive || flat || !conv_in)) {
+        ctx->err = "msm: the endomorphism path needs a sort and a table conversion of its own";
+        return K16_ERR_ARG;
+    }
+    if ((rc = msm_sort_plan(ctx, SL, d_scalars, n, c, flat, reuse, conv_in, conv_out, &sa, glv))) return rc;
     sa.remap        = ctx->remap_next;
     ctx->remap_next = nullptr;
     sa.skip         = skip;
@@ -1956,14 +2123,14 @@
         K16_HIP(ctx, hipEventRecord(L.sort_done, st));
         K16_HIP(ctx, hipStreamWaitEvent(k16_lane_stream(ctx, derive_lane), L.sort_done, 0));
     } else if (!reuse) {
-        const k16_ctx::Lane::GraphKey key{0, d_scalars, n, c, seg, flat ? 1u : 0u, sa.hs[0] ? 1 : 0};
+        const k16_ctx::Lane::GraphKey key{0, d_scalars, n, c, seg, (flat ? 1u : 0u) | (glv ? 2u : 0u), sa.hs[0] ? 1 : 0};
         rc = sort_graphs ? run_graph_section(ctx, L, st, key, sort_body) : sort_body();
         if (rc) return rc;
-        L.sorted_scalars         = d_scalars;
+        L.sorted_scalars         = glv ? nullptr : d_scalars;
         L.sorted_n               = n;
         L.sorted_c               = c;
         L.sorted_skip            = skip;
-        L.sorted_plain_partition = msm_sort_is_plain_partition(ctx, n, c, flat, skip);
+        L.sorted_plain_partition = !glv && msm_sort_is_plain_partition(ctx, n, c, flat, skip);
         K16_HIP(ctx, hipEventRecord(L.sort_done, st));
     }
     tk.tick("sorted");
@@ -2040,7 +2207,7 @@
     };
     {
         const k16_ctx::Lane::GraphKey key{1 + (int)sizeof(typename E::Pt), (const void*)&SL, n, c,
-                                          seg * 64u + mlog, flat ? 1u : 0u, ctx->enq_slot};
+                                          seg * 64u + mlog, (flat ? 1u : 0u) | (glv ? 2u : 0u), ctx->enq_slot};
         return use_graphs ? run_graph_section(ctx, L, st, key, tail_body) : tail_body();
     }
 }
diff --git a/keyless-zk-proofs_amd/k16.py b/keyless-zk-proofs_amd/k16.py
--- a/keyless-zk-proofs_amd/k16.py
+++ b/keyless-zk-proofs_amd/k16.py
@@ -29,7 +29,7 @@
     "k16_runtime_hw_queues", "k16_device_count", "k16_host_threads", "k16_ctx_create", "k16_ctx_create_ex", "k16_ctx_destroy", "k16_last_error", "k16_sync", "k16_stream",
     "k16_dev_alloc", "k16_dev_free", "k16_h2d", "k16_d2h", "k16_host_register", "k16_host_unregister",
     "k16_timer_start", "k16_timer_stop", "k16_kernel_stats_enable", "k16_kernel_stats_reset", "k16_kernel_stats_get",
-    "k16_ctx_set_option", "k16_msm", "k16_msm_host", "k16_msm_enqueue", "k16_msm_finish", "k16_msm_finish_group", "k16_msm_pending", "k16_msm_abort_all", "k16_msm_bases_prepare", "k16_msm_enqueue_prepared", "k16_msm_fixed_base_info", "k16_msm_fixed_base_prepare", "k16_msm_enqueue_fixed_base", "k16_msm_set_window_bits", "k16_msm_set_lane", "k16_points_sum",
+    "k16_ctx_set_option", "k16_msm", "k16_msm_host", "k16_msm_enqueue", "k16_msm_finish", "k16_msm_finish_group", "k16_msm_pending", "k16_msm_abort_all", "k16_msm_bases_prepare", "k16_msm_enqueue_prepared", "k16_msm_fixed_base_info", "k16_msm_fixed_base_prepare", "k16_msm_enqueue_fixed_base", "k16_msm_set_window_bits", "k16_msm_uses_endomorphism", "k16_msm_set_lane", "k16_points_sum",
     "k16_msm_zero_row_mask", "k16_msm_set_zero_row_mask", "k16_msm_sort_from_lane", "k16_scalar_classes_create", "k16_scalar_classes_destroy", "k16_scalar_classes_build", "k16_scalar_classes_counts", "k16_msm_enqueue_classified",
     "k16_ntt", "k16_ntt_host", "k16_synth_points", "k16_synth_points_scalars", "k16_field_op_vec", "k16_point_op_vec", "k16_coop_exec",
     "k16_prover_create", "k16_prover_create_mem", "k16_prover_create_shared", "k16_prover_destroy", "k16_prover_info",
@@ -105,6 +105,7 @@
     L.k16_msm_fixed_base_prepare.argtypes = [vp, i32, vp, u64, vp]
     L.k16_msm_enqueue_fixed_base.argtypes = [vp, i32, vp, vp, u64]
     L.k16_msm_set_window_bits.argtypes = [vp, u32]
+    L.k16_msm_uses_endomorphism.argtypes = [vp, i32, u64, C.POINTER(u64), C.POINTER(u64)]
     L.k16_msm_set_lane.argtypes = [vp, i32]
     L.k16_points_sum.argtypes = [i32, vp, u64, vp, vp]
     L.k16_msm_zero_row_mask.argtypes = [vp, i32, vp, u64, vp]
@@ -324,6 +325,13 @@
     def set_window_bits(self, c):
         self._chk(self.L.k16_msm_set_window_bits(self.h, c))
 
+    def msm_uses_endomorphism(self, group, n):
+        lo, hi = C.c_uint64(0), C.c_uint64(0)
+        rc = self.L.k16_msm_uses_endomorphism(self.h, group, n, C.byref(lo), C.byref(hi))
+        if rc < 0:
+            self._chk(rc)
+        return bool(rc), lo.value, hi.value
+
     def msm_device(self, group, d_bases, d_scalars, n):
         x = np.zeros(XYZZ_BYTES[group], dtype=np.uint8)
         a = np.zeros(AFF_BYTES[group], dtype=np.uint8)
```

After: 763.0 million points/s. -2.9%, worse.
